# ecmwf/anemoi-models

Measured on AMD Instinct MI355X. Metric: mesh-node updates/sec (fwd step), higher is better.
Workload: dtype bf16; 1 GPU; N320->ico-6, 16 GT blocks, 1024 ch, batch 1, 2 x 90 input vars -> 80 output vars, full encoder+processor+decoder forward; mesh_nodes=40962, grid_nodes=542080, processor_blocks=16, rollout_steps=1, parallelism=single GPU, device=AMD Radeon Graphics

## Files before the change

anemoi_models_amd/_lib.py:

```python

from __future__ import annotations

import ctypes
import os
from ctypes import c_char_p
from ctypes import c_float
from ctypes import c_int
from ctypes import c_int64
from ctypes import c_uint32
from ctypes import c_void_p

import torch

_PKG_DIR = os.path.dirname(os.path.abspath(__file__))
LIB_PATH = os.path.join(_PKG_DIR, "lib", "libanemoi_amd.so")

ANEMOI_OK = 0
ANEMOI_ERR_INVALID = 1
ANEMOI_ERR_UNSUPPORTED = 2
ANEMOI_ERR_LAUNCH = 3

F32 = 0
BF16 = 1
I32 = 2
U8 = 3

ACT_NONE, ACT_GELU, ACT_SILU, ACT_RELU = 0, 1, 2, 3
ACT_CODES = {"Identity": ACT_NONE, "GELU": ACT_GELU, "SiLU": ACT_SILU, "ReLU": ACT_RELU}

LOSS_MSE, LOSS_MAE, LOSS_HUBER, LOSS_LOGCOSH = 0, 1, 2, 3
LOSS_KINDS = {"mse": LOSS_MSE, "mae": LOSS_MAE, "huber": LOSS_HUBER, "logcosh": LOSS_LOGCOSH}

ENS_AFCRPS, ENS_MEAN_SE, ENS_VARIANCE = 0, 1, 2
ENS_KINDS = {"afcrps": ENS_AFCRPS, "mean_se": ENS_MEAN_SE, "variance": ENS_VARIANCE}
ENS_MAX_MEMBERS = 16

COND_LN_MAX_K = 32


def cond_ln_padded_k(k: int) -> int:
    return 4 if k <= 4 else (8 if k <= 8 else (16 if k <= 16 else 32))


ABI_VERSION = 55

LINEAR_ENTRIES = {"linear": 0, "ln": 1, "stats": 2, "dual": 3, "actgrad": 4, "batched": 5}
LINEAR_KERNEL_NONE, LINEAR_KERNEL_128, LINEAR_KERNEL_PERSISTENT = 0, 1, 2
LINEAR_REST_NONE, LINEAR_REST_IN_LAUNCH, LINEAR_REST_SKINNY, LINEAR_REST_128 = 0, 1, 2, 3


class LinearArgs(ctypes.Structure):

    _fields_ = [
        ("struct_bytes", c_int64),
        ("entry", ctypes.c_int32), ("dtype", ctypes.c_int32), ("out_dtype", ctypes.c_int32), ("act", ctypes.c_int32),
        ("x", c_void_p), ("w", c_void_p), ("bias", c_void_p), ("colsum", c_void_p), ("stats", c_void_p),
        ("residual", c_void_p), ("y", c_void_p),
        ("ldx", c_int64), ("ldr", c_int64), ("ldy", c_int64), ("M", c_int64),
        ("N", ctypes.c_int32), ("K", ctypes.c_int32),
        ("workspace", c_void_p), ("workspace_bytes", c_int64), ("stats_out", c_void_p),
        ("stride_x", c_int64), ("stride_w", c_int64), ("stride_y", c_int64),
        ("batch", ctypes.c_int32), ("reserved", ctypes.c_int32),
    ]


class LinearRouteLaunch(ctypes.Structure):

    _fields_ = [
        ("row0", c_int64), ("rows", c_int64), ("tiles", c_int64),
        ("mh", ctypes.c_int32), ("blocks", ctypes.c_int32), ("tail_rows", ctypes.c_int32),
        ("stagger_phases", ctypes.c_int32), ("stagger_unit", ctypes.c_int32), ("reserved", ctypes.c_int32),
    ]


class LinearRoute(ctypes.Structure):

    _fields_ = [
        ("struct_bytes", c_int64),
        ("kernel", ctypes.c_int32), ("n_launches", ctypes.c_int32),
        ("launch", LinearRouteLaunch * 2),
        ("main_rows", c_int64),
        ("rest", ctypes.c_int32), ("nt", ctypes.c_int32),
        ("rest_row0", c_int64), ("rest_rows", c_int64), ("rs_rows", c_int64),
        ("vec_ok", ctypes.c_int32), ("split", ctypes.c_int32), ("model", ctypes.c_int32), ("reserved", ctypes.c_int32),
    ]


def linear_route(entry: str, **fields):
    args, route = LinearArgs(), LinearRoute()
    args.struct_bytes, route.struct_bytes = ctypes.sizeof(LinearArgs), ctypes.sizeof(LinearRoute)
    args.entry = LINEAR_ENTRIES[entry]
    for name, value in fields.items():
        setattr(args, name, value)
    return load().anemoi_linear_route(ctypes.byref(args), ctypes.byref(route)), route


class GtBlockArgs(ctypes.Structure):

    _fields_ = [
        ("struct_bytes", c_int64), ("n_dst", c_int64),
        ("dtype", ctypes.c_int32), ("C", ctypes.c_int32), ("H", ctypes.c_int32), ("up", ctypes.c_int32),
        ("hidden", ctypes.c_int32), ("act", ctypes.c_int32), ("k_proj", ctypes.c_int32), ("n_in", ctypes.c_int32),
        ("eps_mlp", c_float), ("eps_out", c_float),
        ("x", c_void_p), ("ldx", c_int64), ("x_stats", c_void_p),
        ("w_in", c_void_p), ("b_in", c_void_p), ("cs_in", c_void_p),
        ("sq", c_void_p), ("ld_sq", c_int64),
        ("q", c_void_p), ("k", c_void_p), ("v", c_void_p), ("x_r", c_void_p), ("u", c_void_p),
        ("ldq", c_int64), ("ldkv", c_int64), ("ldr", c_int64), ("ldu", c_int64),
        ("edge_attr", c_void_p), ("rowptr", c_void_p), ("col", c_void_p),
        ("att", c_void_p), ("ld_att", c_int64),
        ("w_proj", c_void_p), ("b_proj", c_void_p), ("res", c_void_p), ("ld_res", c_int64), ("y", c_void_p),
        ("y_stats", c_void_p),
        ("w_fc1", c_void_p), ("b_fc1", c_void_p), ("cs_fc1", c_void_p), ("h", c_void_p),
        ("w_fc2", c_void_p), ("b_fc2", c_void_p), ("out", c_void_p), ("out_stats", c_void_p),
        ("stats_ws", c_void_p), ("stats_ws_bytes", c_int64),
        ("run_ptr", c_void_p), ("run_perm", c_void_p), ("n_runs", c_int64),
        ("sched", c_void_p), ("sched_slots", ctypes.c_int32), ("sched_steps", ctypes.c_int32), ("n_src", c_int64),
        ("run_dst", c_void_p), ("n_edges", c_int64),
        ("tile_hdr", c_void_p), ("tile_dst", c_void_p), ("tile_src", c_void_p), ("tile_slot", c_void_p), ("tile_xcd", c_void_p),
        ("tile_max_per_xcd", ctypes.c_int32), ("tile_src_cap", ctypes.c_int32), ("tile_edge_cap", ctypes.c_int32),
        ("tile_pad", ctypes.c_int32),
    ]

class TfmBlockArgs(ctypes.Structure):

    _fields_ = [
        ("struct_bytes", c_int64), ("rows", c_int64),
        ("dtype", ctypes.c_int32), ("B", ctypes.c_int32), ("S", ctypes.c_int32), ("C", ctypes.c_int32), ("H", ctypes.c_int32),
        ("hidden", ctypes.c_int32), ("act", ctypes.c_int32), ("window", ctypes.c_int32),
        ("eps1", c_float), ("eps2", c_float),
        ("dropout_p", c_float), ("dropout_seed", c_uint32), ("dropout_seed_dev", c_void_p),
        ("dropout_h0", ctypes.c_int32), ("dropout_h_total", ctypes.c_int32),
        ("x", c_void_p), ("ldx", c_int64),
        ("ln1_w", c_void_p), ("ln1_b", c_void_p), ("ln2_w", c_void_p), ("ln2_b", c_void_p),
        ("w_qkv", c_void_p), ("b_qkv", c_void_p), ("w_proj", c_void_p), ("b_proj", c_void_p),
        ("w_fc1", c_void_p), ("b_fc1", c_void_p), ("w_fc2", c_void_p), ("b_fc2", c_void_p),
        ("h_ln", c_void_p), ("qkv", c_void_p), ("att", c_void_p), ("y", c_void_p), ("h", c_void_p),
        ("mhsa_ws", c_void_p), ("out", c_void_p),
    ]


OPT_MAX_TENSORS = 88
OPT_CHUNK = 4096
OPT_CONSTS = 8
OPT_SKIP_ALL = 3
OPT_SUMSQ_DEPTH = OPT_CHUNK // 256 + 6 + 3


class MultiTensorArgs(ctypes.Structure):

    _fields_ = [
        ("struct_bytes", c_int64), ("n_tensors", c_int64),
        ("numel", c_void_p), ("params", c_void_p), ("grads", c_void_p), ("exp_avg", c_void_p), ("exp_avg_sq", c_void_p),
        ("workspace", c_void_p), ("workspace_floats", c_int64), ("sumsq", c_void_p), ("consts", c_void_p), ("coef", c_void_p),
        ("beta1", ctypes.c_double), ("beta2", ctypes.c_double), ("eps", ctypes.c_double),
    ]


class AdamwConstantsArgs(ctypes.Structure):

    _fields_ = [
        ("struct_bytes", c_int64), ("n_groups", c_int64),
        ("step", c_void_p), ("lr_dev", c_void_p), ("lr", c_void_p), ("beta1", c_void_p), ("beta2", c_void_p),
        ("weight_decay", c_void_p), ("sumsq", c_void_p), ("skipped", c_void_p), ("consts", c_void_p),
        ("max_norm", c_float), ("has_max_norm", ctypes.c_int32), ("skip_nonfinite", ctypes.c_int32),
        ("reserved", ctypes.c_int32),
    ]


AVERAGE_EMA, AVERAGE_SWA = 0, 1
AVG_CONSTS = 4
LR_MAX_GROUPS = 32


class AverageConstantsArgs(ctypes.Structure):

    _fields_ = [
        ("struct_bytes", c_int64), ("n_averaged", c_void_p), ("step", c_void_p), ("skip", c_void_p), ("avg", c_void_p),
        ("decay", ctypes.c_double), ("start_step", c_int64), ("every", c_int64),
        ("kind", ctypes.c_int32), ("use_warmup", ctypes.c_int32),
    ]


class MultiAverageArgs(ctypes.Structure):

    _fields_ = [
        ("struct_bytes", c_int64), ("n_tensors", c_int64), ("numel", c_void_p), ("params", c_void_p), ("shadow", c_void_p),
        ("avg", c_void_p),
    ]


class MultiSwapArgs(ctypes.Structure):

    _fields_ = [("struct_bytes", c_int64), ("n_tensors", c_int64), ("numel", c_void_p), ("a", c_void_p), ("b", c_void_p)]


class LrScheduleArgs(ctypes.Structure):

    _fields_ = [
        ("struct_bytes", c_int64), ("n_groups", c_int64), ("step", c_void_p), ("lr", c_void_p), ("base", c_void_p),
        ("lr_min", c_void_p), ("warmup_start", c_void_p), ("warmup_steps", c_void_p), ("total_steps", c_void_p),
        ("warmup_prefix", c_void_p),
    ]


SIGNATURES = {
    "anemoi_abi_version": (c_int, []),
    "anemoi_build_info": (ctypes.c_char_p, []),
    "anemoi_last_error": (c_char_p, []),
    "anemoi_layer_norm": (c_int, [c_int, c_void_p, c_int64, c_void_p, c_void_p, c_void_p, c_int64, c_int64, c_int,
                                  c_float, c_void_p]),
    "anemoi_layer_norm_residual": (c_int, [c_int, c_void_p, c_int64, c_void_p, c_void_p, c_void_p, c_int64, c_void_p, c_int64,
                                           c_int64, c_int, c_float, c_void_p]),
    "anemoi_layer_norm_stats": (c_int, [c_int, c_void_p, c_int64, c_void_p, c_void_p, c_void_p, c_int64, c_void_p, c_int64,
                                        c_int, c_float, c_void_p]),
    "anemoi_linear": (c_int, [c_int, c_int, c_void_p, c_int64, c_void_p, c_void_p, c_void_p, c_int64, c_void_p,
                              c_int64, c_int64, c_int, c_int, c_int, c_void_p]),
    "anemoi_linear_stats": (c_int, [c_int, c_void_p, c_int64, c_void_p, c_void_p, c_void_p, c_void_p, c_void_p, c_int64,
                                    c_void_p, c_int64, c_int64, c_int, c_int, c_void_p, c_int64, c_float, c_void_p,
                                    c_void_p]),
    "anemoi_row_stats": (c_int, [c_int, c_void_p, c_int64, c_void_p, c_int64, c_int, c_float, c_void_p]),
    "anemoi_linear_ln": (c_int, [c_int, c_int, c_void_p, c_int64, c_void_p, c_void_p, c_void_p, c_void_p, c_void_p,
                                 c_int64, c_void_p, c_int64, c_int64, c_int, c_int, c_int, c_void_p]),
    "anemoi_edge_attr_csr": (c_int, [c_void_p, c_int, c_void_p, c_int, c_int64, c_void_p, c_void_p, c_int, c_int,
                                     c_int64, c_void_p]),
    "anemoi_gt_edge_attention_folded": (c_int, [c_int, c_void_p, c_int64, c_void_p, c_void_p, c_int64, c_void_p,
                                                c_int64, c_void_p, c_int64, c_void_p, c_int, c_void_p, c_void_p,
                                                c_void_p, c_int64, c_void_p, c_int64, c_int, c_int, c_void_p]),
    "anemoi_gt_edge_attention_raw": (c_int, [c_void_p, c_int64, c_void_p, c_int64, c_void_p, c_void_p, c_int64, c_void_p,
                                             c_int, c_void_p, c_void_p, c_void_p, c_int64, c_void_p, c_int64, c_int64,
                                             c_int, c_int, c_int, c_int, c_void_p]),
    "anemoi_gt_edge_attention_folded_runs": (c_int, [c_int, c_void_p, c_int64, c_void_p, c_void_p, c_int64, c_void_p,
                                                     c_int64, c_void_p, c_int64, c_void_p, c_int, c_void_p, c_void_p,
                                                     c_void_p, c_void_p, c_int64, c_void_p, c_int64, c_void_p, c_int64, c_int,
                                                     c_int, c_void_p]),
    "anemoi_gt_edge_attention_folded_groups": (c_int, [c_int, c_void_p, c_int64, c_void_p, c_void_p, c_int64, c_void_p,
                                                       c_int64, c_void_p, c_int64, c_void_p, c_int, c_void_p, c_void_p,
                                                       c_void_p, c_void_p, c_void_p, c_int64, c_int64, c_void_p, c_int64,
                                                       c_void_p, c_int64, c_int, c_int, c_void_p]),
    "anemoi_edge_schedule_shape": (c_int, [c_int, c_int64, c_int, c_void_p, c_void_p]),
    "anemoi_gt_edge_attention_folded_sched": (c_int, [c_int, c_void_p, c_int64, c_void_p, c_void_p, c_int64, c_void_p,
                                                      c_int64, c_void_p, c_int64, c_void_p, c_int, c_void_p, c_void_p,
                                                      c_void_p, c_int, c_int, c_int64, c_int64, c_void_p, c_int64, c_void_p,
                                                      c_int64, c_int, c_int, c_void_p]),
    "anemoi_gt_edge_attention_folded_tiles": (c_int, [c_int, c_void_p, c_int64, c_void_p, c_void_p, c_int64, c_void_p,
                                                      c_int64, c_void_p, c_int64, c_void_p, c_int, c_void_p, c_void_p,
                                                      c_void_p, c_void_p, c_void_p, c_void_p, c_void_p, c_int, c_int, c_int,
                                                      c_int64, c_int64, c_void_p, c_int64, c_void_p, c_int64, c_int, c_int,
                                                      c_void_p]),
    "anemoi_linear_dual": (c_int, [c_int, c_void_p, c_int64, c_void_p, c_void_p, c_void_p, c_int64, c_void_p, c_int64,
                                   c_int64, c_int, c_int, c_int, c_void_p]),
    "anemoi_linear_route": (c_int, [ctypes.POINTER(LinearArgs), ctypes.POINTER(LinearRoute)]),
    "anemoi_linear_actgrad": (c_int, [c_int, c_void_p, c_int64, c_void_p, c_void_p, c_int64, c_void_p, c_int64, c_int64,
                                      c_int, c_int, c_int, c_void_p]),
    "anemoi_gt_conv": (c_int, [c_int, c_void_p, c_int64, c_void_p, c_void_p, c_int64, c_void_p, c_int64, c_void_p, c_int64,
                               c_void_p, c_void_p, c_void_p, c_int64, c_void_p, c_int64, c_int, c_int, c_float, c_uint32,
                               c_void_p, c_void_p]),
    "anemoi_gt_conv_backward_dst": (c_int, [c_int, c_void_p, c_int64, c_void_p, c_void_p, c_int64, c_void_p, c_int64,
                                            c_void_p, c_int64, c_void_p, c_void_p, c_void_p, c_void_p, c_void_p, c_void_p,
                                            c_void_p, c_int64, c_int64, c_int, c_int, c_float, c_uint32, c_void_p,
                                            c_void_p]),
    "anemoi_gt_conv_backward_src": (c_int, [c_int, c_void_p, c_int64, c_void_p, c_int64, c_void_p, c_void_p, c_void_p,
                                            c_void_p, c_void_p, c_void_p, c_void_p, c_void_p, c_int64, c_void_p, c_int64,
                                            c_int64, c_int, c_int, c_float, c_uint32, c_void_p, c_void_p]),
    "anemoi_gt_edge_attention": (c_int, [c_int, c_void_p, c_int64, c_void_p, c_void_p, c_int64, c_void_p, c_int64,
                                         c_void_p, c_int, c_int, c_void_p, c_void_p, c_void_p, c_void_p, c_void_p,
                                         c_int64, c_int64, c_int, c_int, c_void_p]),
    "anemoi_gather_add_act": (c_int, [c_int, c_void_p, c_int64, c_void_p, c_int64, c_void_p, c_int64, c_void_p, c_void_p,
                                      c_void_p, c_int64, c_int64, c_int, c_int, c_void_p]),
    "anemoi_segment_sum": (c_int, [c_int, c_void_p, c_int64, c_void_p, c_void_p, c_int64, c_int64, c_int, c_void_p]),
    "anemoi_segment_sum_cat": (c_int, [c_int, c_void_p, c_int64, c_void_p, c_void_p, c_int64, c_void_p, c_int64, c_int64,
                                       c_int, c_void_p]),
    "anemoi_mhsa_workspace_bytes": (c_int64, [c_int, c_int, c_int, c_int, c_int]),
    "anemoi_mhsa": (c_int, [c_int, c_void_p, c_int64, c_void_p, c_int64, c_void_p, c_void_p, c_int, c_int, c_int, c_int,
                            c_int, c_float, c_uint32, c_void_p, c_int, c_int, c_void_p]),
    "anemoi_mhsa_backward_workspace_bytes": (c_int64, [c_int, c_int, c_int, c_int, c_int]),
    "anemoi_mhsa_backward": (c_int, [c_int, c_void_p, c_int64, c_void_p, c_int64, c_void_p, c_int64, c_void_p, c_void_p,
                                     c_void_p, c_int64, c_void_p, c_int, c_int, c_int, c_int, c_int, c_float, c_uint32,
                                     c_void_p, c_int, c_int, c_void_p]),
    "anemoi_assemble_nodes": (c_int, [c_int, c_void_p, c_int, c_int, c_int, c_int64, c_int, c_void_p, c_int,
                                      c_void_p, c_int, c_void_p, c_int64, c_void_p, c_void_p, c_void_p]),
    "anemoi_finalize_output": (c_int, [c_void_p, c_int, c_void_p, c_int, c_int, c_int, c_int64, c_int, c_void_p,
                                       c_void_p, c_void_p, c_void_p, c_void_p, c_void_p]),
    "anemoi_assemble_node_rows": (c_int, [c_int, c_void_p, c_int, c_int64, c_int, c_void_p, c_int, c_void_p, c_int,
                                          c_void_p, c_int64, c_void_p, c_int64, c_void_p, c_void_p, c_void_p]),
    "anemoi_finalize_output_rows": (c_int, [c_void_p, c_int, c_void_p, c_int, c_int64, c_int, c_void_p, c_void_p, c_int64,
                                            c_void_p, c_void_p, c_void_p, c_void_p, c_void_p]),
    "anemoi_bound_output": (c_int, [c_void_p, c_int, c_int64, c_int, c_void_p, c_void_p, c_void_p, c_void_p, c_int,
                                    c_void_p, c_void_p, c_void_p, c_void_p]),
    "anemoi_prognostic_residual": (c_int, [c_void_p, c_int, c_void_p, c_int, c_int, c_int, c_int64, c_int, c_void_p,
                                           c_void_p, c_int, c_void_p]),
    "anemoi_advance_input": (c_int, [c_void_p, c_int, c_int, c_int, c_int64, c_int, c_void_p, c_int, c_void_p, c_int,
                                     c_void_p, c_void_p]),
    "anemoi_advance_state": (c_int, [c_void_p, c_void_p, c_int, c_int, c_int, c_int64, c_int, c_void_p, c_int, c_void_p,
                                     c_int, c_void_p, c_void_p]),
    "anemoi_advance_state_backward": (c_int, [c_void_p, c_void_p, c_void_p, c_int, c_int, c_int, c_int64, c_int, c_int,
                                              c_void_p, c_void_p, c_int, c_void_p]),
    "anemoi_assemble_nodes_backward": (c_int, [c_int, c_void_p, c_int64, c_void_p, c_int, c_int, c_int, c_int64, c_int,
                                               c_void_p]),
    "anemoi_prognostic_residual_backward": (c_int, [c_void_p, c_int, c_void_p, c_int, c_int, c_int, c_int64, c_int,
                                                    c_void_p, c_void_p]),
    "anemoi_csr_project": (c_int, [c_void_p, c_int64, c_int64, c_int64, c_void_p, c_int64, c_int64, c_int64, c_int, c_int,
                                   c_int64, c_int64, c_void_p, c_void_p, c_void_p, c_void_p, c_void_p, c_int, c_void_p,
                                   c_void_p, c_int, c_void_p]),
    "anemoi_weighted_mse_workspace_floats": (c_int64, [c_int64, c_int]),
    "anemoi_weighted_mse": (c_int, [c_void_p, c_void_p, c_int64, c_int, c_int64, c_void_p, c_void_p, c_void_p, c_float,
                                    c_void_p, c_void_p, c_int64, c_void_p]),
    "anemoi_weighted_mse_backward": (c_int, [c_void_p, c_void_p, c_int64, c_int, c_int64, c_void_p, c_void_p, c_void_p,
                                             c_float, c_void_p, c_void_p, c_void_p]),
    "anemoi_weighted_error_workspace_floats": (c_int64, [c_int64, c_int64, c_int]),
    "anemoi_weighted_error": (c_int, [c_int, c_float, c_void_p, c_void_p, c_int64, c_int, c_int64, c_int64, c_void_p, c_void_p,
                                      c_void_p, c_void_p, c_float, c_void_p, c_void_p, c_int64, c_void_p]),
    "anemoi_weighted_error_backward": (c_int, [c_int, c_float, c_void_p, c_void_p, c_int64, c_int, c_int64, c_int64, c_void_p,
                                               c_void_p, c_void_p, c_void_p, c_float, c_void_p, c_void_p, c_void_p]),
    "anemoi_ensemble_score_workspace_floats": (c_int64, [c_int64, c_int64, c_int, c_int]),
    "anemoi_ensemble_score": (c_int, [c_int, c_float, c_void_p, c_void_p, c_int64, c_int, c_int64, c_int, c_int64, c_void_p,
                                      c_void_p, c_void_p, c_void_p, c_float, c_void_p, c_void_p, c_int64, c_void_p]),
    "anemoi_ensemble_score_backward": (c_int, [c_int, c_float, c_void_p, c_void_p, c_int64, c_int, c_int64, c_int, c_int64,
                                               c_void_p, c_void_p, c_void_p, c_void_p, c_float, c_void_p, c_void_p, c_void_p]),
    "anemoi_cond_layer_norm": (c_int, [c_int, c_void_p, c_int64, c_void_p, c_int64, c_int, c_void_p, c_int64, c_void_p, c_void_p,
                                       c_void_p, c_void_p, c_int64, c_void_p, c_int64, c_int, c_float, c_void_p]),
    "anemoi_cond_layer_norm_backward_workspace_floats": (c_int64, [c_int64, c_int, c_int]),
    "anemoi_cond_layer_norm_backward": (c_int, [c_int, c_void_p, c_int64, c_void_p, c_int64, c_void_p, c_void_p, c_int64, c_int,
                                                c_void_p, c_int64, c_void_p, c_void_p, c_void_p, c_int64, c_void_p, c_void_p, c_void_p,
                                                c_void_p, c_void_p, c_int64, c_int, c_void_p, c_int64, c_void_p]),
    "anemoi_gaussian_noise": (c_int, [c_void_p, c_int64, c_int, c_float, c_uint32, c_void_p, c_void_p]),
    "anemoi_transpose": (c_int, [c_int, c_void_p, c_int64, c_void_p, c_int64, c_int64, c_int, c_void_p]),
    "anemoi_transpose_colsum_rows": (c_int64, [c_int64, c_int64]),
    "anemoi_transpose_chunked": (c_int, [c_int, c_void_p, c_int64, c_void_p, c_int64, c_int64, c_int, c_int64, c_void_p,
                                         c_void_p]),
    "anemoi_weight_grad_tn": (c_int, [c_void_p, c_int64, c_void_p, c_int64, c_void_p, c_int64, c_void_p, c_int64, c_int64,
                                      c_int, c_int, c_int, c_void_p]),
    "anemoi_linear_batched": (c_int, [c_int, c_int, c_void_p, c_int64, c_int64, c_void_p, c_int64, c_void_p, c_int64,
                                      c_int64, c_int, c_int64, c_int, c_int, c_void_p]),
    "anemoi_col_sum_workspace_floats": (c_int64, [c_int64, c_int]),
# ... 97 lines not shown
```

anemoi_models_amd/layers/block.py:

```python

from __future__ import annotations

import os
from abc import ABC
from abc import abstractmethod
from typing import Optional

import torch
from torch import Tensor
from torch import nn

from .. import ops
from .. import runtime
from .. import training
from ..runtime import EdgePlan
from .conv import GraphConv
from .conv import GraphTransformerConv
from .mlp import MLP
from .mlp import NativeSequential
from .mlp import activation_class
from .mlp import fused_activation_name
from .mlp import linear_native
from .normalization import ConditionalLayerNorm


def inference_num_chunks() -> int:
    return int(os.environ.get("ANEMOI_INFERENCE_NUM_CHUNKS", "1"))


def _group_size(group) -> int:
    return 1 if group is None else group.size()


def _as_compute(x: Tensor, dtype: torch.dtype) -> Tensor:
    x = x if x.dtype == dtype else x.to(dtype)
    return x if (x.dim() == 2 and x.stride(1) == 1) else x.contiguous()



def folded_edge_phase(q: Tensor, k: Tensor, v: Tensor, x_r: Optional[Tensor], u: Tensor, edge_attr_csr: Tensor, plan,
                      num_heads: int, up: int, ld_out: Optional[int] = None) -> Tensor:
    lists = runtime.edge_lists(plan, q.dtype, q.shape[-1], num_heads, up)
    return ops.gt_edge_attention_folded(q, k, v, x_r, u, edge_attr_csr, plan.rowptr, plan.col, num_heads, up, ld_out=ld_out,
                                        **lists._asdict())


class EmbeddedRows:

    def __init__(self, x_aug: Tensor, one_col: int, emb: nn.Linear, h: Optional[Tensor], packed, tag: str) -> None:
        self.x_aug, self.one_col, self.emb, self.h, self._packed, self._tag = x_aug, one_col, emb, h, packed, tag

    @property
    def dtype(self) -> torch.dtype:
        return self.x_aug.dtype

    @property
    def device(self) -> torch.device:
        return self.x_aug.device

    @property
    def shape(self):
        return (self.x_aug.shape[0], self.emb.out_features)

    def stats(self, eps: float) -> Tensor:
        if self.h is not None:
            return ops.row_stats(self.h, eps)
        kp = self.x_aug.shape[1]
        t = self._packed.get((self._tag, "embstats", self.dtype, kp, self.one_col), [self.emb.weight, self.emb.bias],
                             lambda: runtime.embedding_stats_operator(self.emb.weight, self.emb.bias, kp, self.one_col,
                                                                      self.dtype))
        return ops.row_stats(runtime.linear(self.x_aug, t, None, stats_eps=eps), eps)


class BaseBlock(nn.Module, ABC):

    @abstractmethod
    def forward(self, x, edge_attr, edge_index, shapes, batch_size, size=None, model_comm_group=None): ...


class GraphTransformerBaseBlock(BaseBlock, ABC):

    def __init__(
        self,
        in_channels: int,
        hidden_dim: int,
        out_channels: int,
        edge_dim: int,
        num_heads: int = 16,
        bias: bool = True,
        activation: str = "GELU",
        num_chunks: int = 1,
        update_src_nodes: bool = False,
        **kwargs,
    ) -> None:
        super().__init__(**kwargs)
        self.update_src_nodes = update_src_nodes
        self.out_channels_conv = out_channels // num_heads
        self.num_heads = num_heads
        self.num_chunks = num_chunks
        self.activation = activation
        self.edge_dim = edge_dim
        width = num_heads * self.out_channels_conv

        self.lin_key = nn.Linear(in_channels, width)
        self.lin_query = nn.Linear(in_channels, width)
        self.lin_value = nn.Linear(in_channels, width)
        self.lin_self = nn.Linear(in_channels, width, bias=bias)
        self.lin_edge = nn.Linear(edge_dim, width)
        self.conv = GraphTransformerConv(out_channels=self.out_channels_conv)
        self.projection = nn.Linear(out_channels, out_channels)

        act = activation_class(activation)
        self.node_dst_mlp = nn.Sequential(
            nn.LayerNorm(out_channels), nn.Linear(out_channels, hidden_dim), act(), nn.Linear(hidden_dim, out_channels)
        )
        self.layer_norm1 = nn.LayerNorm(in_channels)
        if self.update_src_nodes:
            self.node_src_mlp = nn.Sequential(
                nn.LayerNorm(out_channels), nn.Linear(out_channels, hidden_dim), act(),
                nn.Linear(hidden_dim, out_channels),
            )
        self._packed = runtime.PackedWeights()
        self._plans = runtime.PlanCache()
        self._dst_mlp: Optional[NativeSequential] = None
        self._src_mlp: Optional[NativeSequential] = None

    def shard_qkve_heads(self, query: Tensor, key: Tensor, value: Tensor, edges: Tensor, shapes: tuple, batch_size: int,
                         model_comm_group=None):
        h, d = self.num_heads, self.out_channels_conv
        if _group_size(model_comm_group) <= 1:
            return tuple(t.reshape(t.shape[0], h, d) for t in (query, key, value, edges))
        from ..distributed.transformer import shard_heads

        assert batch_size == 1, "Only batch size of 1 is supported when model is sharded across GPUs"
        shapes_src, shapes_dst, shapes_edges = shapes
        out = []
        for t, shp in ((query, shapes_dst), (key, shapes_src), (value, shapes_src), (edges, shapes_edges)):
            t = t.reshape(1, t.shape[0], h, d).permute(0, 2, 1, 3)
            t = shard_heads(t, shapes=shp, mgroup=model_comm_group)
            out.append(t[0].permute(1, 0, 2).contiguous())
        return tuple(out)

    def shard_output_seq(self, out: Tensor, shapes: tuple, batch_size: int, model_comm_group=None) -> Tensor:
        if _group_size(model_comm_group) <= 1:
            return out.reshape(out.shape[0], -1)
        from ..distributed.transformer import shard_sequence

        t = out.permute(1, 0, 2).unsqueeze(0)
        t = shard_sequence(t, shapes=shapes[1], mgroup=model_comm_group)
        return t[0].permute(1, 0, 2).reshape(t.shape[2], -1).contiguous()

    def _cat_linear(self, tag: str, layers, dtype):
        w = self._packed.get((tag, "w", dtype), [l.weight for l in layers],
                             lambda: runtime.pack_weight([l.weight for l in layers], dtype))
# ... 405 lines not shown
            n_own = x_src.shape[0]
            kv = torch.empty((n_own + halo.n_recv, 2 * c), dtype=dtype, device=x_src.device)
            self._ln_linear(xs, *kv_args, out=kv[:n_own])
            pending = halo.start(kv, n_own)
        del xs
        xd = self._ln_begin(self.layer_norm2, x_dst)
        up = self.fold_width(dtype)
        if up is not None:
            wp, bp = self._folded_out(dtype, up)
            sq = self._ln_linear(xd, "squ", lambda: self._folded_in("squ", sq_layers, dtype, up),
                                 lambda: self._folded_rows(sq_layers, up),
                                 self._fold_params(sq_layers))
            del xd
            if halo is not None:
                halo.finish(pending)
            if num_chunks <= 1 and not self.update_src_nodes and not mx:
                new_dst = self._folded_tail(sq[:, c:2 * c], kv[:, :c], kv[:, c:], sq[:, :c], sq[:, 2 * c:], edge_attr_csr, plan,
                                            h_dst, up, out_stats_eps)
                return (x_src.h if isinstance(x_src, EmbeddedRows) else x_src), new_dst
            att = folded_edge_phase(sq[:, c:2 * c], kv[:, :c], kv[:, c:], sq[:, :c], sq[:, 2 * c:], edge_attr_csr, plan,
                                    self.num_heads, up, ld_out=wp.shape[1])
        else:
            if halo is not None:
                raise NotImplementedError("node-partitioned blocks need the folded edge kernel")
            wp, bp = self._cat_linear("proj", [self.projection], dtype)
            we, be = self._edge_params()
            sq = self._ln_linear(xd, "sq", lambda: self._cat_linear("sq", sq_layers, dtype),
                                 lambda: self._cat_rows(sq_layers),
                                 [l.weight for l in sq_layers] + [l.bias for l in sq_layers])
            del xd
            att = self.conv.fused(sq[:, c:], kv[:, :c], kv[:, c:], sq[:, :c], edge_attr_csr, self.edge_dim, we, be,
                                  plan, self.num_heads)
        del sq, kv
        y = runtime.linear(att, wp, bp, residual=h_dst,
                       stats_eps=self._mlp_ln_eps("dst", dtype) if num_chunks <= 1 else None)
        del att
        if mx:
            new_dst = self._mx_node_mlp(y, "dst", num_chunks)
        else:
            new_dst = self._node_mlp(y, "dst", num_chunks, out_stats_eps=out_stats_eps)
        if isinstance(x_src, EmbeddedRows):
            x_src = x_src.h
        new_src = self._node_mlp(x_src, "src", num_chunks) if self.update_src_nodes else x_src
        return new_src, new_dst

    RAW_ROWS_DEFAULT = "1"

    def _raw_source_weights(self, x_src, dtype):
        h, d = self.num_heads, self.out_channels_conv
        if (not isinstance(x_src, EmbeddedRows) or x_src.h is not None or self.update_src_nodes
                or dtype != torch.bfloat16 or not x_src.x_aug.is_cuda
                or os.environ.get("ANEMOI_AMD_EDGE_RAW", self.RAW_ROWS_DEFAULT) == "0"):
            return None
        ks, k_in = x_src.x_aug.shape[1], x_src.emb.in_features
        sum_col = ks - 1 if x_src.one_col != ks - 1 else ks - 2
        if self.fold_width(dtype) is None or h != 16 or ks not in (64, 128, 256) or sum_col < k_in:
            return None
        kv_layers = [self.lin_key, self.lin_value]
        ln, emb = self.layer_norm1, x_src.emb

        def build():
            f, b, _ = runtime.fold_embedded_layer_norm(*self._cat_rows(kv_layers), ln.weight, ln.bias, emb.weight,
                                                       emb.bias, ks, x_src.one_col, torch.float32)
            c = h * d
            w_qt = f[:c].view(h, d, ks).transpose(1, 2)
            w_g = f[c:].view(h, d, ks).clone()
            w_g[:, :, sum_col] = b[c:].view(h, d)
            if d % ops.k_multiple(dtype) != 0:
                w_qt, w_g = torch.block_diag(*w_qt), torch.block_diag(*w_g)
            return w_qt.to(dtype).contiguous(), w_g.to(dtype).contiguous(), sum_col

        return self._packed.get(("kv", "rawrows", dtype, ks, x_src.one_col, x_src._tag),
                                [l.weight for l in kv_layers] + [l.bias for l in kv_layers]
                                + [ln.weight, ln.bias, emb.weight, emb.bias], build)

    def _native_raw_sources(self, x_src, src_stats: Tensor, x_dst, h_dst: Tensor, edge_attr_csr: Tensor, plan, raw,
                            out_stats_eps: Optional[float]) -> Tensor:
        dtype = x_dst.dtype
        c, h = self.num_heads * self.out_channels_conv, self.num_heads
        w_qt, w_g, sum_col = raw
        up = self.fold_width(dtype)
        sq_layers = [self.lin_self, self.lin_query]
        wp, bp = self._folded_out(dtype, up)
        sq = self._ln_linear(self._ln_begin(self.layer_norm2, x_dst), "squ",
                             lambda: self._folded_in("squ", sq_layers, dtype, up),
                             lambda: self._folded_rows(sq_layers, up), self._fold_params(sq_layers))
        per_head = w_qt.dim() == 3
        qt = ops.linear_heads(sq[:, c:2 * c], w_qt) if per_head else runtime.linear(sq[:, c:2 * c], w_qt)
        att = torch.empty((sq.shape[0], wp.shape[1]), dtype=dtype, device=sq.device)
        if wp.shape[1] > c + h * up:
            att[:, c + h * up:].zero_()
        g = ops.gt_edge_attention_raw(qt, x_src.x_aug, src_stats, sq[:, 2 * c:2 * c + h * up], edge_attr_csr, plan.rowptr,
                                      plan.col, h, self.out_channels_conv, up, sum_col, att[:, c:c + h * up])
        del qt
        if per_head:
            ops.linear_heads(g, w_g, out=att[:, :c])
            ops.add(att[:, :c], sq[:, :c], out=att[:, :c])
        else:
            runtime.linear(g, w_g, residual=sq[:, :c], out=att[:, :c])
        del g
        del sq
        y = runtime.linear(att, wp, bp, residual=h_dst, stats_eps=self._mlp_ln_eps("dst", dtype))
        del att
        return self._node_mlp(y, "dst", 1, out_stats_eps=out_stats_eps)

    def _sharded(self, x, edge_attr: Tensor, edge_index: Tensor, shapes: tuple, batch_size: int, model_comm_group, size=None):
        from .. import autograd

        x_src, x_dst = x
        dtype = runtime.compute_dtype(x_dst)
        x_src, x_dst = _as_compute(x_src, dtype), _as_compute(x_dst, dtype)
        ln1, ln2 = self.layer_norm1, self.layer_norm2
        hs = autograd.layer_norm(x_src, ln1.weight, ln1.bias, ln1.eps)
        hd = autograd.layer_norm(x_dst, ln2.weight, ln2.bias, ln2.eps)
        x_r = autograd.linear(hd, self.lin_self.weight, self.lin_self.bias)
        q = autograd.linear(hd, self.lin_query.weight, self.lin_query.bias)
        k = autograd.linear(hs, self.lin_key.weight, self.lin_key.bias)
        v = autograd.linear(hs, self.lin_value.weight, self.lin_value.bias)
        e = autograd.linear(_as_compute(edge_attr, dtype), self.lin_edge.weight, self.lin_edge.bias)
        q, k, v, e = self.shard_qkve_heads(q, k, v, e, shapes, batch_size, model_comm_group)
        out = self.conv(q, k, v, e, edge_index, size=size)
        out = self.shard_output_seq(out, shapes, batch_size, model_comm_group)
        out = autograd.linear(out + x_r, self.projection.weight, self.projection.bias, "Identity", x_dst)
        new_src = training.sequential(self.node_src_mlp, x_src, residual=x_src) if self.update_src_nodes else x_src
        return new_src, training.sequential(self.node_dst_mlp, out, residual=out)

    def forward(
        self,
        x,
        edge_attr: Tensor,
        edge_index: Tensor,
        shapes: tuple,
        batch_size: int,
        model_comm_group=None,
        size=None,
    ):
        if _group_size(model_comm_group) > 1:
            assert batch_size == 1, "Only batch size of 1 is supported when model is sharded across GPUs"
            return self._sharded(x, edge_attr, edge_index, shapes, batch_size, model_comm_group, size), edge_attr
        if training.wants_grad(self, x[0], x[1], edge_attr):
            return training.gt_mapper_block(self, x, edge_attr, edge_index, size)
        x_src, x_dst = x
        dtype = runtime.compute_dtype(x_dst)
        n_src, n_dst = x_src.shape[0], x_dst.shape[0]
        if size is not None and tuple(size) != (n_src, n_dst):
            raise ValueError(f"Encountered tensors with sizes {(n_src, n_dst)}, but expected size {tuple(size)}")
        plan, ea = self._edge_inputs(edge_attr, edge_index, n_src, n_dst, dtype)
        num_chunks = self.num_chunks if self.training else inference_num_chunks()
        new_src, new_dst = self.native(_as_compute(x_src, dtype), _as_compute(x_dst, dtype), ea, plan, num_chunks)
        return (new_src if self.update_src_nodes else x[0], new_dst), edge_attr


class GraphConvBaseBlock(BaseBlock, ABC):
    def __init__(
        self,
        in_channels: int,
        out_channels: int,
        mlp_extra_layers: int = 0,
        activation: str = "SiLU",
        update_src_nodes: bool = True,
        num_chunks: int = 1,
        **kwargs,
    ) -> None:
        super().__init__(**kwargs)
        self.update_src_nodes = update_src_nodes
        self.num_chunks = num_chunks
        self.node_mlp = MLP(2 * in_channels, out_channels, out_channels, n_extra_layers=mlp_extra_layers,
                            activation=activation)
        self.conv = GraphConv(in_channels=in_channels, out_channels=out_channels, mlp_extra_layers=mlp_extra_layers,
                              activation=activation)
        self._packed = runtime.PackedWeights()
        self._plans = runtime.PlanCache()

    @abstractmethod
    def forward(self, x, edge_attr: Tensor, edge_index: Tensor, shapes: tuple, model_comm_group=None, size=None):
        """``(new nodes, new edge state)`` -- reference layers/block.py:157-167."""

    @staticmethod
    def _check_width(width: int, dtype) -> None:
        mult = ops.k_multiple(dtype)
# ... 307 lines not shown
```

anemoi_models_amd/layers/mapper.py:

```python

from __future__ import annotations

from abc import ABC
from typing import Optional

import numpy as np
import torch
from torch import Tensor
from torch import nn

from .. import ops
from .. import runtime
from .. import training
from .block import EmbeddedRows
from .block import GraphConvMapperBlock
from .block import GraphTransformerMapperBlock
from .block import inference_num_chunks
from .graph import TrainableTensor
from .mlp import MLP
from .mlp import linear_native


class BaseMapper(nn.Module, ABC):
    def __init__(self, in_channels_src: int = 0, in_channels_dst: int = 0, hidden_dim: int = 128,
# ... 31 lines not shown
        xin = x if x.dtype == dtype else x.to(dtype)
        return NativeSequential(seq)(xin if xin.stride(-1) == 1 else xin.contiguous())

    def pre_process(self, x, shard_shapes, model_comm_group=None):
        shapes_src, shapes_dst = shard_shapes
        x_src, x_dst = x
        return x_src, x_dst, shapes_src, shapes_dst

    def post_process(self, x_dst, shapes_dst, model_comm_group=None):
        return x_dst


class ForwardMapperPreProcessMixin:

    def pre_process(self, x, shard_shapes, model_comm_group=None):
        from ..distributed.shapes import change_channels_in_shape

        from ..distributed.graph import shard_tensor

        x_src, x_dst, shapes_src, shapes_dst = super().pre_process(x, shard_shapes, model_comm_group)
        x_src = shard_tensor(x_src, 0, shapes_src, model_comm_group)
        x_dst = shard_tensor(x_dst, 0, shapes_dst, model_comm_group)
        return (self._apply_module(self.emb_nodes_src, x_src), self._apply_module(self.emb_nodes_dst, x_dst),
                change_channels_in_shape(shapes_src, self.hidden_dim), change_channels_in_shape(shapes_dst, self.hidden_dim))


class BackwardMapperPostProcessMixin:

    def post_process(self, x_dst, shapes_dst, model_comm_group=None):
        from ..distributed.graph import gather_tensor
        from ..distributed.shapes import change_channels_in_shape

        x_dst = self._apply_module(self.node_data_extractor, x_dst)
        return gather_tensor(x_dst, 0, change_channels_in_shape(shapes_dst, self.out_channels_dst), model_comm_group)


class GraphEdgeMixin:

    def _register_edges(self, sub_graph, edge_attributes, src_size: int, dst_size: int, trainable_size: int) -> None:
        assert sub_graph, f"{self.__class__.__name__} needs a valid sub_graph to register edges."
        assert edge_attributes is not None, "Edge attributes must be provided"
        attr = torch.cat([sub_graph[name] for name in edge_attributes], dim=1)
        self.edge_dim = attr.shape[1] + trainable_size
        self.register_buffer("edge_attr", attr, persistent=False)
        self.register_buffer("edge_index_base", sub_graph.edge_index, persistent=False)
        self.register_buffer("edge_inc", torch.from_numpy(np.asarray([[src_size], [dst_size]], dtype=np.int64)),
                             persistent=True)

    def _expand_edges(self, edge_index: Tensor, edge_inc: Tensor, batch_size: int) -> Tensor:
        return runtime.expand_edges(edge_index, edge_inc, batch_size)


class GraphTransformerBaseMapper(GraphEdgeMixin, BaseMapper):
    def __init__(
        self,
        in_channels_src: int = 0,
        in_channels_dst: int = 0,
        hidden_dim: int = 128,
        trainable_size: int = 8,
        out_channels_dst: Optional[int] = None,
        num_chunks: int = 1,
        cpu_offload: bool = False,
        activation: str = "GELU",
        num_heads: int = 16,
        mlp_hidden_ratio: int = 4,
        sub_graph=None,
        sub_graph_edge_attributes: Optional[list] = None,
        src_grid_size: int = 0,
        dst_grid_size: int = 0,
    ) -> None:
        super().__init__(in_channels_src, in_channels_dst, hidden_dim, out_channels_dst=out_channels_dst,
                         num_chunks=num_chunks, cpu_offload=cpu_offload, activation=activation)
        self._register_edges(sub_graph, sub_graph_edge_attributes, src_grid_size, dst_grid_size, trainable_size)
        self.trainable = TrainableTensor(trainable_size=trainable_size, tensor_size=self.edge_attr.shape[0])
        self.proc = GraphTransformerMapperBlock(
            hidden_dim, mlp_hidden_ratio * hidden_dim, hidden_dim, num_heads=num_heads, edge_dim=self.edge_dim,
            activation=activation, num_chunks=num_chunks,
        )
        self.offload_layers(cpu_offload)
        self.emb_nodes_dst = nn.Linear(self.in_channels_dst, self.hidden_dim)
        self._packed = runtime.PackedWeights()
        self._plans = runtime.PlanCache()

    def _embed(self, x_src: Tensor, x_dst: Tensor, one_cols=(None, None)):
        return x_src, x_dst

    def _embedded(self, tag: str, lin: nn.Linear, x: Tensor, eps: Optional[float], one_col: Optional[int],
                  materialise: bool):
        k_in = lin.in_features
        if eps is None or not runtime.embed_fold_enabled(x.dtype) or 2 * (k_in + 1) > lin.out_features:
            return linear_native(self._packed, tag, lin, x, stats_eps=eps)
        if one_col is None:
            kp = ops.round_up(k_in + 1, ops.k_multiple(x.dtype))
            xa = torch.zeros((x.shape[0], kp), dtype=x.dtype, device=x.device)
            xa[:, :k_in].copy_(x[:, :k_in])
            xa[:, k_in].fill_(1.0)
            x, one_col = xa, k_in
        elif not (k_in <= one_col < x.shape[1]):
            raise ValueError(f"{tag}: constant-1 column {one_col} outside the K padding [{k_in}, {x.shape[1]})")
        h = linear_native(self._packed, tag, lin, x, stats_eps=eps) if materialise else None
        return EmbeddedRows(x, one_col, lin, h, self._packed, tag)

    def _extract(self, x_dst: Tensor, out_dtype) -> Tensor:
        return x_dst

    def _block_ln_eps(self, dtype):
        if not runtime.ln_fold_enabled(dtype):
            return None, None
        return self.proc.layer_norm1.eps, self.proc.layer_norm2.eps

    def _extract_ln_eps(self, dtype) -> Optional[float]:
        ext = getattr(self, "node_data_extractor", None)
        if isinstance(ext, nn.Sequential) and isinstance(ext[0], nn.LayerNorm) and runtime.ln_fold_enabled(dtype):
            return ext[0].eps
        return None

    def native(self, x_src: Tensor, x_dst: Tensor, batch_size: int, out_dtype: Optional[torch.dtype] = None,
               src_map: Optional[Tensor] = None, dst_map: Optional[Tensor] = None, one_cols=(None, None)) -> Tensor:
        n_src, n_dst = x_src.shape[0], x_dst.shape[0]
        plan = self._plans.get(self.edge_index_base, n_src, n_dst, batch_size, self.edge_inc, src_map, dst_map)
        ea = runtime.edge_attr_csr_cached(self._packed, self.edge_attr, self.trainable.trainable, plan,
                                          *self.proc.edge_layout(x_dst.dtype))
        h_src, h_dst = self._embed(x_src, x_dst, one_cols)
        num_chunks = self.proc.num_chunks if self.training else inference_num_chunks()
        _, h_dst = self.proc.native(h_src, h_dst, ea, plan, num_chunks, out_stats_eps=self._extract_ln_eps(h_dst.dtype))
        return self._extract(h_dst, out_dtype)

    def native_local(self, x_src: Tensor, x_dst: Tensor, local_graph, out_dtype: Optional[torch.dtype] = None,
                     one_cols=(None, None)) -> Tensor:
        plan = local_graph.plan
        ea = runtime.edge_attr_csr_cached(self._packed, self.edge_attr, self.trainable.trainable, plan,
                                          *self.proc.edge_layout(x_dst.dtype))
        h_src, h_dst = self._embed(x_src, x_dst, one_cols)
        num_chunks = self.proc.num_chunks if self.training else inference_num_chunks()
        _, h_dst = self.proc.native(h_src, h_dst, ea, plan, num_chunks, local_graph.halo,
                                    out_stats_eps=self._extract_ln_eps(h_dst.dtype))
        return self._extract(h_dst, out_dtype)

    def _run_sharded(self, x, batch_size: int, shard_shapes, model_comm_group) -> Tensor:
        from ..distributed.graph import shard_tensor
        from ..distributed.shapes import get_shape_shards

        size = (sum(s_[0] for s_ in shard_shapes[0]), sum(s_[0] for s_ in shard_shapes[1]))
        edge_attr = self.trainable(self.edge_attr, batch_size)
        edge_index = self._expand_edges(self.edge_index_base, self.edge_inc, batch_size)
        shapes_edge_attr = get_shape_shards(edge_attr, 0, model_comm_group)
        edge_attr = shard_tensor(edge_attr, 0, shapes_edge_attr, model_comm_group)
        x_src, x_dst, shapes_src, shapes_dst = self.pre_process(x, shard_shapes, model_comm_group)
        (x_src, x_dst), edge_attr = self.proc((x_src, x_dst), edge_attr, edge_index, (shapes_src, shapes_dst, shapes_edge_attr),
                                              batch_size, model_comm_group, size=size)
        return self.post_process(x_dst, shapes_dst, model_comm_group)

    def _run(self, x, batch_size: int, shard_shapes, model_comm_group) -> Tensor:
        if model_comm_group is not None and model_comm_group.size() > 1:
            assert batch_size == 1, "Only batch size of 1 is supported when model is sharded across GPUs"
            return self._run_sharded(x, batch_size, shard_shapes, model_comm_group)
        x_src, x_dst = x
        if shard_shapes is not None:
            size = (sum(s[0] for s in shard_shapes[0]), sum(s[0] for s in shard_shapes[1]))
            if size != (x_src.shape[0], x_dst.shape[0]):
                raise ValueError(f"shard_shapes describe {size} nodes, inputs have {(x_src.shape[0], x_dst.shape[0])}")
        if training.wants_grad(self, x_src, x_dst):
            with self._offloaded():
                return training.gt_mapper(self, x_src, x_dst, batch_size)
        dtype = runtime.compute_dtype(x_dst)

        def prep(t):
            t = t if t.dtype == dtype else t.to(dtype)
            return t if t.stride(-1) == 1 else t.contiguous()

        return self.native(prep(x_src), prep(x_dst), batch_size)

    def forward(self, x, batch_size: int, shard_shapes, model_comm_group=None) -> Tensor:
        return self._run(x, batch_size, shard_shapes, model_comm_group)


class GraphTransformerForwardMapper(ForwardMapperPreProcessMixin, GraphTransformerBaseMapper):

    def __init__(self, in_channels_src: int = 0, in_channels_dst: int = 0, hidden_dim: int = 128,
                 trainable_size: int = 8, out_channels_dst: Optional[int] = None, num_chunks: int = 1,
                 cpu_offload: bool = False, activation: str = "GELU", num_heads: int = 16, mlp_hidden_ratio: int = 4,
                 sub_graph=None, sub_graph_edge_attributes: Optional[list] = None, src_grid_size: int = 0,
                 dst_grid_size: int = 0) -> None:
        super().__init__(in_channels_src, in_channels_dst, hidden_dim, trainable_size,
                         out_channels_dst=out_channels_dst, num_chunks=num_chunks, cpu_offload=cpu_offload,
                         activation=activation, num_heads=num_heads, mlp_hidden_ratio=mlp_hidden_ratio,
                         sub_graph=sub_graph, sub_graph_edge_attributes=sub_graph_edge_attributes,
                         src_grid_size=src_grid_size, dst_grid_size=dst_grid_size)
        self.emb_nodes_src = nn.Linear(self.in_channels_src, self.hidden_dim)

    def _embed(self, x_src: Tensor, x_dst: Tensor, one_cols=(None, None)):
        eps1, eps2 = self._block_ln_eps(x_src.dtype)
        return (self._embedded("emb_nodes_src", self.emb_nodes_src, x_src, eps1, one_cols[0],
                               materialise=self.proc.update_src_nodes),
                self._embedded("emb_nodes_dst", self.emb_nodes_dst, x_dst, eps2, one_cols[1], materialise=True))

    def forward(self, x, batch_size: int, shard_shapes, model_comm_group=None):
        x_dst = self._run(x, batch_size, shard_shapes, model_comm_group)
        return x[0], x_dst


class GraphTransformerBackwardMapper(BackwardMapperPostProcessMixin, GraphTransformerBaseMapper):

    def __init__(self, in_channels_src: int = 0, in_channels_dst: int = 0, hidden_dim: int = 128,
                 trainable_size: int = 8, out_channels_dst: Optional[int] = None, num_chunks: int = 1,
                 cpu_offload: bool = False, activation: str = "GELU", num_heads: int = 16, mlp_hidden_ratio: int = 4,
                 sub_graph=None, sub_graph_edge_attributes: Optional[list] = None, src_grid_size: int = 0,
                 dst_grid_size: int = 0) -> None:
        super().__init__(in_channels_src, in_channels_dst, hidden_dim, trainable_size,
                         out_channels_dst=out_channels_dst, num_chunks=num_chunks, cpu_offload=cpu_offload,
                         activation=activation, num_heads=num_heads, mlp_hidden_ratio=mlp_hidden_ratio,
                         sub_graph=sub_graph, sub_graph_edge_attributes=sub_graph_edge_attributes,
                         src_grid_size=src_grid_size, dst_grid_size=dst_grid_size)
        self.node_data_extractor = nn.Sequential(nn.LayerNorm(self.hidden_dim),
                                                 nn.Linear(self.hidden_dim, self.out_channels_dst))
        self.proc.mx_node_mlp = False

    def pre_process(self, x, shard_shapes, model_comm_group=None):
        from ..distributed.shapes import change_channels_in_shape

        from ..distributed.graph import shard_tensor

        x_src, x_dst, shapes_src, shapes_dst = super().pre_process(x, shard_shapes, model_comm_group)
        x_dst = shard_tensor(x_dst, 0, shapes_dst, model_comm_group)
        return (x_src, self._apply_module(self.emb_nodes_dst, x_dst), change_channels_in_shape(shapes_src, self.hidden_dim),
                change_channels_in_shape(shapes_dst, self.hidden_dim))

    def _embed(self, x_src: Tensor, x_dst: Tensor, one_cols=(None, None)):
        return x_src, self._embedded("emb_nodes_dst", self.emb_nodes_dst, x_dst, self._block_ln_eps(x_dst.dtype)[1],
                                     one_cols[1], materialise=True)

    def _extract(self, x_dst: Tensor, out_dtype) -> Tensor:
        ln, lin = self.node_data_extractor[0], self.node_data_extractor[1]
        if runtime.ln_fold_enabled(x_dst.dtype) and x_dst.shape[1] % ops.k_multiple(x_dst.dtype) == 0:
            wf, bf, cs = self._packed.get(("extract", "lnfold", x_dst.dtype), [lin.weight, lin.bias, ln.weight, ln.bias],
                                          lambda: runtime.fold_layer_norm(lin.weight.detach().float(), lin.bias,
                                                                          ln.weight, ln.bias, x_dst.dtype))
            return runtime.linear(x_dst, wf, bf, out_dtype=out_dtype, ln=(ops.row_stats(x_dst, ln.eps), cs))
        h = ops.layer_norm(x_dst, runtime.f32c(ln.weight), runtime.f32c(ln.bias), ln.eps)
        return linear_native(self._packed, "extract", lin, h, out_dtype=out_dtype)

    def forward(self, x, batch_size: int, shard_shapes, model_comm_group=None) -> Tensor:
        return self._run(x, batch_size, shard_shapes, model_comm_group)


class GNNBaseMapper(GraphEdgeMixin, BaseMapper):
    def __init__(self, in_channels_src: int = 0, in_channels_dst: int = 0, hidden_dim: int = 128,
                 trainable_size: int = 8, out_channels_dst: Optional[int] = None, num_chunks: int = 1,
                 cpu_offload: bool = False, activation: str = "SiLU", mlp_extra_layers: int = 0, sub_graph=None,
                 sub_graph_edge_attributes: Optional[list] = None, src_grid_size: int = 0,
                 dst_grid_size: int = 0) -> None:
        super().__init__(in_channels_src, in_channels_dst, hidden_dim, out_channels_dst=out_channels_dst,
                         num_chunks=num_chunks, cpu_offload=cpu_offload, activation=activation)
        self._register_edges(sub_graph, sub_graph_edge_attributes, src_grid_size, dst_grid_size, trainable_size)
        self.emb_edges = MLP(in_features=self.edge_dim, hidden_dim=hidden_dim, out_features=hidden_dim,
                             n_extra_layers=mlp_extra_layers, activation=activation)
        self.trainable = TrainableTensor(trainable_size=trainable_size, tensor_size=self.edge_attr.shape[0])
        self._plans = runtime.PlanCache()

    def prepare_edges(self, size, batch_size: int, model_comm_group=None):
        from ..distributed.graph import shard_tensor
        from ..distributed.khop_edges import sort_edges_1hop_sharding

        edge_attr = self.trainable(self.edge_attr, batch_size)
        edge_index = self._expand_edges(self.edge_index_base, self.edge_inc, batch_size)
        if model_comm_group is not None and model_comm_group.size() > 1:
            edge_attr, edge_index, shapes_edge_attr, shapes_edge_idx = sort_edges_1hop_sharding(size, edge_attr, edge_index,
                                                                                                model_comm_group)
            edge_index = shard_tensor(edge_index, 1, shapes_edge_idx, model_comm_group)
            edge_attr = shard_tensor(edge_attr, 0, shapes_edge_attr, model_comm_group)
        return self.emb_edges(edge_attr), edge_index

    def _embed(self, x_src: Tensor, x_dst: Tensor):
        return x_src, x_dst

    def _extract(self, x_dst: Tensor, out_dtype) -> Tensor:
        return x_dst

    def native(self, x_src: Tensor, x_dst: Tensor, batch_size: int, out_dtype: Optional[torch.dtype] = None,
               src_map: Optional[Tensor] = None, dst_map: Optional[Tensor] = None):
        n_src, n_dst = x_src.shape[0], x_dst.shape[0]
        plan = self._plans.get(self.edge_index_base, n_src, n_dst, batch_size, self.edge_inc, src_map, dst_map)
        dtype = x_dst.dtype
        ea = ops.edge_attr_csr(self.edge_attr, self.trainable.trainable, plan.perm)
        e = ops.convert_pad(ea[:, : self.edge_dim], dtype, ops.round_up(self.edge_dim, ops.k_multiple(dtype)))
        e = self.emb_edges.native()(e)
        h_src, h_dst = self._embed(x_src, x_dst)
        (h_src, h_dst), _ = self.proc.native(h_src, h_dst, e, plan)
        return h_src, self._extract(h_dst, out_dtype)

    def native_local(self, x_src: Tensor, x_dst: Tensor, local_graph, out_dtype: Optional[torch.dtype] = None,
                     x_src_extra: Optional[Tensor] = None):
        plan = local_graph.plan
        dtype = x_dst.dtype
        ea = ops.edge_attr_csr(self.edge_attr, self.trainable.trainable, plan.perm)
        e = ops.convert_pad(ea[:, : self.edge_dim], dtype, ops.round_up(self.edge_dim, ops.k_multiple(dtype)))
        e = self.emb_edges.native()(e)
        h_src, h_dst = self._embed(x_src, x_dst)
        (_, h_dst), _ = self.proc.native(h_src, h_dst, e, plan, local_graph.halo)
        extra = None
        if x_src_extra is not None:
            hx = self.emb_nodes_src.native()(x_src_extra) if hasattr(self, "emb_nodes_src") else x_src_extra
            c = hx.shape[1]
            if self.proc.update_src_nodes:
                xcat = torch.empty((hx.shape[0], 2 * c), dtype=dtype, device=hx.device)
                xcat[:, :c].copy_(hx)
                xcat[:, c:].copy_(hx)
                hx = self.proc.node_mlp.native()(xcat, residual=hx)
            extra = hx
        return extra, self._extract(h_dst, out_dtype)

    def _run(self, x, batch_size: int, shard_shapes, model_comm_group):
        if model_comm_group is not None and model_comm_group.size() > 1:
            assert batch_size == 1, "Only batch size of 1 is supported when model is sharded across GPUs"
            size = (sum(s_[0] for s_ in shard_shapes[0]), sum(s_[0] for s_ in shard_shapes[1]))
            edge_attr, edge_index = self.prepare_edges(size, batch_size, model_comm_group)
            x_src, x_dst, shapes_src, shapes_dst = self.pre_process(x, shard_shapes, model_comm_group)
            (x_src, x_dst), _ = self.proc((x_src, x_dst), edge_attr, edge_index, (shapes_src, shapes_dst), model_comm_group,
                                          size=size)
            return x_src, self.post_process(x_dst, shapes_dst, model_comm_group)
        x_src, x_dst = x
# ... 68 lines not shown
```

anemoi_models_amd/models/encoder_processor_decoder.py:

```python

from __future__ import annotations

import logging
from typing import Optional

import torch
from torch import Tensor
from torch import nn

from .. import ops
from .. import runtime
from ..layers.graph import NamedNodesAttributes
from ..layers.truncation import project_add

try:
    from hydra.utils import instantiate as _hydra_instantiate
except ImportError:
    _hydra_instantiate = None

from ..utils.config import instantiate as _local_instantiate
from ..utils.config import REFERENCE_PREFIX

LOGGER = logging.getLogger(__name__)


def instantiate(cfg, **kwargs):
    target = cfg.get("_target_", "") if hasattr(cfg, "get") else ""
    if _hydra_instantiate is not None and not target.startswith(REFERENCE_PREFIX):
        return _hydra_instantiate(cfg, **kwargs)
    return _local_instantiate(cfg, **kwargs)


class AnemoiModelEncProcDec(nn.Module):

    def __init__(self, *, model_config, data_indices, graph_data, truncation_data=None) -> None:
        super().__init__()
        self._graph_data = graph_data
        self._graph_name_data = model_config.graph.data
        self._graph_name_hidden = model_config.graph.hidden

        self._calculate_shapes_and_indices(data_indices)
        self._assert_matching_indices(data_indices)
        self.data_indices = data_indices

        self.multi_step = model_config.training.multistep_input
        self.num_channels = model_config.model.num_channels

        self.node_attributes = NamedNodesAttributes(model_config.model.trainable_parameters.hidden, self._graph_data)
        data, hidden = self._graph_name_data, self._graph_name_hidden
        input_dim = self.multi_step * self.num_input_channels + self.node_attributes.attr_ndims[data]

        self.encoder = instantiate(
            model_config.model.encoder,
            in_channels_src=input_dim,
            in_channels_dst=self.node_attributes.attr_ndims[hidden],
            hidden_dim=self.num_channels,
            sub_graph=self._graph_data[(data, "to", hidden)],
            src_grid_size=self.node_attributes.num_nodes[data],
            dst_grid_size=self.node_attributes.num_nodes[hidden],
        )
        self.processor = instantiate(
            model_config.model.processor,
            num_channels=self.num_channels,
            sub_graph=self._graph_data[(hidden, "to", hidden)],
            src_grid_size=self.node_attributes.num_nodes[hidden],
            dst_grid_size=self.node_attributes.num_nodes[hidden],
            **self._processor_kwargs(model_config),
        )
        self.decoder = instantiate(
            model_config.model.decoder,
            in_channels_src=self.num_channels,
            in_channels_dst=input_dim,
            hidden_dim=self.num_channels,
            out_channels_dst=self.num_output_channels,
            sub_graph=self._graph_data[(hidden, "to", data)],
            src_grid_size=self.node_attributes.num_nodes[hidden],
            dst_grid_size=self.node_attributes.num_nodes[data],
        )
        self.boundings = nn.ModuleList(
            [
                instantiate(cfg, name_to_index=self.data_indices.internal_model.output.name_to_index)
                for cfg in getattr(model_config.model, "bounding", [])
            ]
        )
        self._idx_cache: dict = {}
        self._set_truncation(truncation_data)

    def _set_truncation(self, truncation_data) -> None:
        from ..layers.truncation import TruncationPlan

        plan = TruncationPlan(truncation_data, grid_size=self.node_attributes.num_nodes[self._graph_name_data])
        if plan and len(set(torch.as_tensor(self._internal_input_idx).tolist())) != len(self._internal_input_idx):
            raise ValueError("truncation_data: the prognostic input columns repeat (the input gradient stores each column once)")
        self._truncation = plan if plan else None

    def _calculate_shapes_and_indices(self, data_indices) -> None:
        self.num_input_channels = len(data_indices.internal_model.input)
        self.num_output_channels = len(data_indices.internal_model.output)
        self._internal_input_idx = data_indices.internal_model.input.prognostic
        self._internal_output_idx = data_indices.internal_model.output.prognostic

    def _assert_matching_indices(self, data_indices) -> None:
        n_full = len(data_indices.internal_model.output.full)
        n_diag = len(data_indices.internal_model.output.diagnostic)
        assert len(self._internal_output_idx) == n_full - n_diag, (
            f"Mismatch between the internal data indices ({len(self._internal_output_idx)}) and "
            f"the internal output indices excluding diagnostic variables ({n_full - n_diag})"
        )
        assert len(self._internal_input_idx) == len(
            self._internal_output_idx
        ), f"Internal model indices must match {self._internal_input_idx} != {self._internal_output_idx}"

    def _run_mapper(self, mapper: nn.Module, data, batch_size: int, shard_shapes, model_comm_group=None,
                    use_reentrant: bool = False):
        kwargs = dict(batch_size=batch_size, shard_shapes=shard_shapes, model_comm_group=model_comm_group)
        if not torch.is_grad_enabled():
            return mapper(data, **kwargs)
        from torch.utils.checkpoint import checkpoint

        return checkpoint(mapper, data, **kwargs, use_reentrant=use_reentrant)

    def _processor_kwargs(self, model_config) -> dict:
        return {}

    def _processor_condition(self, batch_size: int, x_latent: Tensor) -> Optional[Tensor]:
        return None

    def _prognostic_indices(self, device):
        key = str(device)
        if key not in self._idx_cache:
            as_i32 = lambda t: torch.as_tensor(t).to(device=device, dtype=torch.int32).contiguous()
            self._idx_cache[key] = (as_i32(self._internal_output_idx), as_i32(self._internal_input_idx))
        return self._idx_cache[key]

    def _mesh_order(self, device):
        key = ("mesh_order", str(device))
        if key not in self._idx_cache:
            latlons = self.node_attributes.latlons(self._graph_name_hidden)
            if not getattr(self, "mesh_locality_order", True):
                order = torch.arange(latlons.shape[0], device=device)
            else:
                order = runtime.locality_order(latlons).to(device)
            self._idx_cache[key] = (order, runtime.inverse_permutation(order))
        return self._idx_cache[key]

    def _with_ones(self, trainable: Optional[Tensor], n_nodes: int, enabled: bool, device=None) -> Optional[Tensor]:
        if not enabled:
            return trainable
        device = trainable.device if trainable is not None else (device or self.node_attributes.latlons(
            self._graph_name_data).device)
        key = ("ones", n_nodes, str(device))
        if key not in self._idx_cache:
            self._idx_cache[key] = torch.ones((n_nodes, 1), dtype=torch.float32, device=device)
        ones = self._idx_cache[key]
        return ones if trainable is None else torch.cat([trainable.detach().float(), ones], dim=1)

    def _embed_fold(self, dtype: torch.dtype) -> bool:
        from ..layers.mapper import GraphTransformerBaseMapper

        return (runtime.embed_fold_enabled(dtype) and isinstance(self.encoder, GraphTransformerBaseMapper)
                and isinstance(self.decoder, GraphTransformerBaseMapper))

    @staticmethod
    def _feature_ld(width: int, dtype: torch.dtype, wide: bool = True) -> int:
        ld = ops.round_up(width, ops.k_multiple(dtype))
        return max(ld, 128) if (wide and dtype == torch.bfloat16) else ld

    @staticmethod
# ... 21 lines not shown
        elif key not in self._idx_cache:
            src = torch.full((self.num_output_channels,), -1, dtype=torch.int32)
            src[torch.as_tensor(self._internal_output_idx).long()] = torch.as_tensor(self._internal_input_idx).to(torch.int32)
            self._idx_cache[key] = src.to(y.device)
        if len(self.boundings) == 0:
            ops.finalize_output(y, x, self._idx_cache[key], input_affine, output_affine, rows=rows)
            return y if y.dtype == out_dtype else y.to(out_dtype)
        plan = self._bounding_plan(y.device, output_affine)
        if plan is None:
            ops.finalize_output(y, x, self._idx_cache[key], input_affine, None, rows=rows)
            if y.dtype != out_dtype:
                y = y.to(out_dtype)
            for bounding in self.boundings:
                y = bounding(y)
            if output_affine is not None:
                y = (y - output_affine[1]) / output_affine[0]
            return y
        op_lists, masked_affine, fin = plan
        ops.finalize_output(y, x, self._idx_cache[key], input_affine, masked_affine, rows=rows)
        ops.bound_output(y, *op_lists, fin=fin)
        return y if y.dtype == out_dtype else y.to(out_dtype)

    def _bounding_plan(self, device, output_affine):
        from ..layers.bounding import bounded_columns
        from ..layers.bounding import compile_boundings

        key = ("boundings", str(device), None if output_affine is None else
               (output_affine[0].data_ptr(), output_affine[0]._version, output_affine[1].data_ptr(),
                output_affine[1]._version))
        if key not in self._idx_cache:
            op_list = compile_boundings(self.boundings)
            if op_list is None:
                self._idx_cache[key] = None
                return None
            lists = (torch.tensor([o[0] for o in op_list], dtype=torch.int32, device=device),
                     torch.tensor([o[1] for o in op_list], dtype=torch.float32, device=device),
                     torch.tensor([o[2] for o in op_list], dtype=torch.float32, device=device),
                     torch.tensor([o[3] for o in op_list], dtype=torch.int32, device=device))
            masked = fin = None
            if output_affine is not None:
                cols = torch.tensor(bounded_columns(op_list), dtype=torch.int64, device=device)
                mul, add = (t.detach().to(device=device, dtype=torch.float32).contiguous() for t in output_affine)
                m_mul, m_add = mul.clone(), add.clone()
                m_mul[cols] = 1.0
                m_add[cols] = 0.0
                masked = (m_mul, m_add)
                fin = (cols.to(torch.int32), mul[cols].contiguous(), add[cols].contiguous())
            self._idx_cache[key] = (lists, masked, fin)
        return self._idx_cache[key]

    def _training_forward(self, x: Tensor, input_affine=None, output_affine=None) -> Tensor:
        from .. import training

        if input_affine is not None or output_affine is not None:
            raise NotImplementedError("input_affine / output_affine belong to the inference interface (predict_step)")
        return training.model_forward(self, x)

    def forward(self, x: Tensor, model_comm_group=None, *, input_affine=None, output_affine=None) -> Tensor:
        if model_comm_group is not None and model_comm_group.size() > 1:
            from ..distributed.partition import sharded_forward

            if getattr(self, "_truncation", None) is not None:
                from ..layers.truncation import REFUSAL

                raise NotImplementedError(REFUSAL)
            return sharded_forward(self, x, model_comm_group, input_affine=input_affine, output_affine=output_affine)
        if torch.is_grad_enabled() and any(p.requires_grad for p in self.parameters()):
            return self._training_forward(x, input_affine, output_affine)
        runtime.require_inference(self)
        batch_size, _, ensemble_size, grid, _ = x.shape
        dtype = runtime.compute_dtype(x)
        kmult = ops.k_multiple(dtype)
        data, hidden = self._graph_name_data, self._graph_name_hidden
        na = self.node_attributes

        width = self.multi_step * self.num_input_channels + na.attr_ndims[data]
        fold = self._embed_fold(dtype)
        tr_data = na.trainable_tensors[data].trainable
        x_data = ops.assemble_nodes(x, na.latlons(data), self._with_ones(tr_data, grid, fold), batch_size, dtype,
                                    ld_out=self._feature_ld(width + int(fold), dtype, fold), in_affine=input_affine)
        order, inv = self._mesh_order(x.device)
        tr_hidden = na.trainable_tensors[hidden].trainable
        w_hidden = na.attr_ndims[hidden]
        x_hidden = ops.assemble_nodes(None, na.latlons(hidden)[order],
                                      self._with_ones(None if tr_hidden is None else tr_hidden[order], order.numel(), fold),
                                      batch_size, dtype, ld_out=self._feature_ld(w_hidden + int(fold), dtype, fold))
        one_data, one_hidden = (width, w_hidden) if fold else (None, None)

        enc = self.encoder.native(x_data, x_hidden, batch_size, dst_map=inv,
                                  **self._one_cols(self.encoder, one_data, one_hidden))
        x_data_latent, x_latent = (x_data, enc) if not isinstance(enc, tuple) else enc
        cond = self._processor_condition(batch_size, x_latent)
        x_proc = (self.processor.native(x_latent, batch_size, node_map=inv) if cond is None
                  else self.processor.native(x_latent, batch_size, node_map=inv, cond=cond))
        x_latent_proc = ops.add(x_proc, x_latent)
        y = self.decoder.native(x_latent_proc, x_data_latent, batch_size, out_dtype=torch.float32, src_map=inv,
                                **self._one_cols(self.decoder, None, one_data if x_data_latent is x_data else None))
        if isinstance(y, tuple):
            y = y[1]

        y = y.view(batch_size, ensemble_size, grid, self.num_output_channels)
        return self._finish(y, x, input_affine, output_affine)
```

anemoi_models_amd/ops.py:

```python

from __future__ import annotations

from typing import NamedTuple
from typing import Optional

import torch
from torch import Tensor

from . import _lib

_DT = {torch.float32: _lib.F32, torch.bfloat16: _lib.BF16}

PROFILE: Optional[list] = None


class _Timed:
    __slots__ = ("name", "work", "start")

    def __init__(self, name: str, **work) -> None:
        self.name, self.work, self.start = name, work, None

    def __enter__(self):
        if PROFILE is not None:
            self.start = torch.cuda.Event(enable_timing=True)
            self.start.record(torch.cuda.current_stream())
        return self

    def __exit__(self, *exc):
        if self.start is not None:
            end = torch.cuda.Event(enable_timing=True)
            end.record(torch.cuda.current_stream())
            PROFILE.append((self.name, self.start, end, self.work))
        return False


def dtype_code(dtype: torch.dtype) -> int:
    try:
        return _DT[dtype]
    except KeyError:
        raise NotImplementedError(f"compute dtype {dtype} is not supported (float32 or bfloat16)") from None


def k_multiple(dtype: torch.dtype) -> int:
    return 128 // torch.empty((), dtype=dtype).element_size()


def round_up(n: int, m: int) -> int:
    return (n + m - 1) // m * m


def _dev(*tensors: Optional[Tensor]) -> None:
    for t in tensors:
        if t is not None and not t.is_cuda:
            raise RuntimeError(
                "anemoi_models_amd kernels run on an MI355X only: got a CPU tensor (there is no CPU fallback)"
            )


_raw_stream = getattr(torch._C, "_cuda_getCurrentRawStream", None)


def _stream() -> int:
    if _raw_stream is not None:
        return _raw_stream(torch.cuda.current_device())
    return torch.cuda.current_stream().cuda_stream


def _rows(t: Tensor) -> Tensor:
    if t.dim() != 2 or (t.shape[1] > 1 and t.stride(1) != 1):
        raise ValueError(f"expected a row-major 2-D tensor (unit inner stride), got shape {tuple(t.shape)} "
                         f"strides {t.stride()}")
    return t


def _ld(t: Tensor) -> int:
    return t.stride(0) if t.shape[0] > 1 else max(t.stride(0), t.shape[1])


def _ptr(t: Optional[Tensor]) -> Optional[int]:
    return None if t is None else t.data_ptr()


def layer_norm(x: Tensor, weight: Tensor, bias: Tensor, eps: float = 1e-5, out: Optional[Tensor] = None,
               residual: Optional[Tensor] = None) -> Tensor:
    _dev(x, weight, bias, out, residual)
    _rows(x)
    if out is None:
        out = torch.empty((x.shape[0], x.shape[1]), dtype=x.dtype, device=x.device)
    if residual is not None and (residual.dtype != x.dtype or residual.shape != x.shape):
        raise ValueError("layer_norm: the residual must have the shape and dtype of x")
    if x.shape[0] == 0:
        return out
    if residual is not None:
        with _Timed("layer_norm", bytes=3 * x.shape[0] * x.shape[1] * x.element_size()):
            st = _lib.load().anemoi_layer_norm_residual(dtype_code(x.dtype), x.data_ptr(), _ld(x), weight.data_ptr(),
                                                        bias.data_ptr(), residual.data_ptr(), _ld(_rows(residual)),
                                                        out.data_ptr(), _ld(_rows(out)), x.shape[0], x.shape[1], eps, _stream())
        _lib.check(st, "anemoi_layer_norm_residual")
        return out
    with _Timed("layer_norm", bytes=2 * x.shape[0] * x.shape[1] * x.element_size()):
        st = _lib.load().anemoi_layer_norm(dtype_code(x.dtype), x.data_ptr(), _ld(x), weight.data_ptr(),
                                           bias.data_ptr(), out.data_ptr(), _ld(_rows(out)), x.shape[0], x.shape[1],
                                           eps, _stream())
    _lib.check(st, "anemoi_layer_norm")
    return out


def layer_norm_with_stats(x: Tensor, weight: Tensor, bias: Tensor, eps: float = 1e-5):
    _dev(x, weight, bias)
    _rows(x)
    out = torch.empty((x.shape[0], x.shape[1]), dtype=x.dtype, device=x.device)
    stats = torch.empty((x.shape[0], 2), dtype=torch.float32, device=x.device)
# ... 264 lines not shown
    if rowptr.dtype != torch.int32 or col.dtype != torch.int32 or rowptr.shape[0] != n_dst + 1:
        raise ValueError("gt_edge_attention: rowptr/col must be int32 with rowptr of length n_dst + 1")
    if col.shape[0] == 0:
        col = torch.zeros(1, dtype=torch.int32, device=q.device)
        edge_attr = torch.zeros((1, max(4, round_up(edge_dim, 4))), dtype=torch.float32, device=q.device)
    alg_bytes = (2 * n_dst + 2 * k.shape[0]) * c * q.element_size() + col.shape[0] * 52 + (n_dst + 1) * 4
    with _Timed("gt_edge_attention", bytes=alg_bytes, n_dst=n_dst, n_src=k.shape[0], edges=col.shape[0]):
        st = _lib.load().anemoi_gt_edge_attention(
            dtype_code(q.dtype), q.data_ptr(), _ld(q), k.data_ptr(), v.data_ptr(), _ld(k), _ptr(x_r),
            0 if x_r is None else _ld(_rows(x_r)), edge_attr.data_ptr(),
            edge_attr.stride(0) if edge_attr.shape[0] > 1 else edge_attr.shape[1], edge_dim, w_edge.data_ptr(),
            b_edge.data_ptr(), rowptr.data_ptr(), col.data_ptr(), out.data_ptr(), _ld(_rows(out)), n_dst, c,
            num_heads, _stream())
    _lib.check(st, "anemoi_gt_edge_attention")
    return out


def gt_edge_attention_folded(q: Tensor, k: Tensor, v: Tensor, x_r: Optional[Tensor], u: Tensor, edge_attr: Tensor,
                             rowptr: Tensor, col: Tensor, num_heads: int, up: int, out: Optional[Tensor] = None,
                             ld_out: Optional[int] = None, lse: Optional[Tensor] = None, runs=None, sched=None,
                             tiles=None) -> Tensor:
    _dev(q, k, v, x_r, u, edge_attr, rowptr, col, out, lse)
    if lse is not None and (lse.dtype != torch.float32 or not lse.is_contiguous()
                            or tuple(lse.shape) != (_rows(q).shape[0], num_heads)):
        raise ValueError("gt_edge_attention_folded: lse must be a contiguous f32 [n_dst, H] tensor")
    n_dst, c = _rows(q).shape
    if _ld(_rows(k)) != _ld(_rows(v)):
        raise ValueError("gt_edge_attention_folded: k and v must share their leading dimension")
    width = c + num_heads * up
    ld = width if ld_out is None else ld_out
    if out is None:
        out = torch.empty((n_dst, ld), dtype=q.dtype, device=q.device)
        if ld > width:
            out[:, width:].zero_()
    if rowptr.dtype != torch.int32 or col.dtype != torch.int32 or rowptr.shape[0] != n_dst + 1:
        raise ValueError("gt_edge_attention_folded: rowptr/col must be int32 with rowptr of length n_dst + 1")
    if edge_attr.shape[0] != col.shape[0] or (col.shape[0] > 0 and (edge_attr.shape[1] != up or
                                                                      not edge_attr.is_contiguous())):
        raise ValueError("gt_edge_attention_folded: edge_attr must be contiguous [E, up]")
    if col.shape[0] == 0:
        col = torch.zeros(1, dtype=torch.int32, device=q.device)
        edge_attr = torch.zeros((1, up), dtype=torch.float32, device=q.device)
    alg_bytes = (2 * n_dst + 2 * k.shape[0]) * c * q.element_size() + col.shape[0] * 52 + (n_dst + 1) * 4
    fused_bytes = alg_bytes + n_dst * ((0 if x_r is None else c) + 2 * num_heads * up) * q.element_size()
    with _Timed("gt_edge_attention", bytes=alg_bytes, fused_bytes=fused_bytes, n_dst=n_dst, n_src=k.shape[0], edges=col.shape[0]):
        lib = _lib.load()
        head = (dtype_code(q.dtype), q.data_ptr(), _ld(q), k.data_ptr(), v.data_ptr(), _ld(_rows(k)), _ptr(x_r),
                0 if x_r is None else _ld(_rows(x_r)), u.data_ptr(), _ld(_rows(u)), edge_attr.data_ptr(), up,
                rowptr.data_ptr(), col.data_ptr())
        tail = (out.data_ptr(), _ld(_rows(out)), _ptr(lse), n_dst, c, num_heads, _stream())
        n_src, n_edges = _rows(k).shape[0], col.shape[0]
        if runs is not None and len(runs) == 3:
            grp_ptr, grp_perm, grp_dst = runs
            _dev(grp_ptr, grp_perm, grp_dst)
            if (grp_ptr.dtype != torch.int32 or grp_perm.dtype != torch.int32 or grp_dst.dtype != torch.int32
                    or grp_perm.shape[0] != n_dst or grp_dst.shape[0] != n_dst):
                raise ValueError("gt_edge_attention_folded: runs = (int32 grp_ptr [n_groups + 1], int32 grp_perm [n_dst], "
                                 "int32 grp_dst [n_dst])")
            st = lib.anemoi_gt_edge_attention_folded_groups(*head, grp_ptr.data_ptr(), grp_dst.data_ptr(), grp_perm.data_ptr(),
                                                            grp_ptr.shape[0] - 1, n_src, *tail)
        elif runs is not None:
            run_ptr, perm = runs
            _dev(run_ptr, perm)
            if run_ptr.dtype != torch.int32 or perm.dtype != torch.int32 or perm.shape[0] != run_ptr.shape[0] - 1:
                raise ValueError("gt_edge_attention_folded: runs = (int32 run_ptr [n_runs + 1], int32 perm [n_runs])")
            st = lib.anemoi_gt_edge_attention_folded_runs(*head, run_ptr.data_ptr(), perm.data_ptr(), run_ptr.shape[0] - 1, *tail)
        elif tiles is not None:
            _dev(tiles.hdr, tiles.dst, tiles.src, tiles.slot, tiles.xcd)
            st = lib.anemoi_gt_edge_attention_folded_tiles(
                *head, tiles.hdr.data_ptr(), tiles.dst.data_ptr(), tiles.src.data_ptr(), tiles.slot.data_ptr(),
                tiles.xcd.data_ptr(), tiles.max_tiles_per_xcd, tiles.src_cap, tiles.edge_cap, n_src, n_edges, *tail)
        elif sched is not None:
            _dev(sched)
            if sched.dtype != torch.int32 or sched.dim() != 3 or sched.shape[0] != 8 or not sched.is_contiguous():
                raise ValueError("gt_edge_attention_folded: sched = contiguous int32 [8, slots, steps]")
            st = lib.anemoi_gt_edge_attention_folded_sched(*head, sched.data_ptr(), sched.shape[1], sched.shape[2], n_src,
                                                           n_edges, *tail)
        else:
            st = lib.anemoi_gt_edge_attention_folded(*head, *tail)
    _lib.check(st, "anemoi_gt_edge_attention_folded")
    return out


def linear_heads(x: Tensor, w: Tensor, out: Optional[Tensor] = None) -> Tensor:
    _dev(x, w, out)
    _rows(x)
    if w.dim() != 3 or w.dtype != x.dtype or not w.is_contiguous():
        raise ValueError("linear_heads: weight must be contiguous [H, N, K] in the activation dtype")
    h, n, k = w.shape
    if x.shape[1] < h * k:
        raise ValueError(f"linear_heads: x has {x.shape[1]} columns, {h} heads of {k} expected")
    if out is None:
        out = torch.empty((x.shape[0], h * n), dtype=x.dtype, device=x.device)
    if _rows(out).shape[1] < h * n or out.dtype != x.dtype or out.shape[0] != x.shape[0]:
        raise ValueError("linear_heads: out must be [M, >= H*N] in the activation dtype")
    m = x.shape[0]
    if m == 0:
        return out
    code = dtype_code(x.dtype)
    with _Timed("linear", flops=2 * m * h * n * k, bytes=(m * h * (k + n) + h * n * k) * x.element_size(), m=m, n=h * n,
                k=k, heads=h):
        st = _lib.load().anemoi_linear_batched(code, code, x.data_ptr(), _ld(x), k, w.data_ptr(), n * k, out.data_ptr(),
                                               _ld(out), n, h, m, n, k, _stream())
    _lib.check(st, "anemoi_linear_batched")
    return out


def gt_edge_attention_raw(qt: Tensor, x_raw: Tensor, src_stats: Tensor, u: Tensor, edge_attr: Tensor, rowptr: Tensor,
                          col: Tensor, num_heads: int, head_dim: int, up: int, sum_col: int, t_out: Tensor,
                          g: Optional[Tensor] = None) -> Tensor:
    _dev(qt, x_raw, src_stats, u, edge_attr, rowptr, col, t_out, g)
    n_dst, ks = _rows(qt).shape[0], _rows(x_raw).shape[1]
    if qt.dtype != torch.bfloat16 or x_raw.dtype != torch.bfloat16 or u.dtype != torch.bfloat16 or t_out.dtype != torch.bfloat16:
        raise NotImplementedError("gt_edge_attention_raw: bf16 only")
    if qt.shape[1] != num_heads * ks:
        raise ValueError(f"gt_edge_attention_raw: qt has {qt.shape[1]} columns, {num_heads} heads of {ks} expected")
    if (src_stats.shape != (x_raw.shape[0], 2) or src_stats.dtype != torch.float32 or not src_stats.is_contiguous()):
        raise ValueError("gt_edge_attention_raw: src_stats must be the contiguous [n_src, 2] f32 result of row_stats")
    if rowptr.dtype != torch.int32 or col.dtype != torch.int32 or rowptr.shape[0] != n_dst + 1:
        raise ValueError("gt_edge_attention_raw: rowptr/col must be int32 with rowptr of length n_dst + 1")
    if edge_attr.shape[0] != col.shape[0] or (col.shape[0] > 0 and (edge_attr.shape[1] != up or
                                                                      not edge_attr.is_contiguous())):
        raise ValueError("gt_edge_attention_raw: edge_attr must be contiguous [E, up]")
    if _rows(u).shape != (n_dst, num_heads * up) or _rows(t_out).shape[0] != n_dst or t_out.shape[1] < num_heads * up:
        raise ValueError("gt_edge_attention_raw: u / t_out must be [n_dst, H*up]")
    if g is None:
        g = torch.empty((n_dst, num_heads * ks), dtype=qt.dtype, device=qt.device)
    if col.shape[0] == 0:
        col = torch.zeros(1, dtype=torch.int32, device=qt.device)
        edge_attr = torch.zeros((1, up), dtype=torch.float32, device=qt.device)
    alg_bytes = (col.shape[0] * (ks * 2 + 4 + up * 4 + 4) + 2 * n_dst * num_heads * ks * 2 + (n_dst + 1) * 4)
    fused_bytes = alg_bytes + n_dst * 2 * num_heads * up * 2
    with _Timed("gt_edge_attention", bytes=alg_bytes, fused_bytes=fused_bytes, n_dst=n_dst, n_src=x_raw.shape[0],
                edges=col.shape[0], raw_rows=ks):
        st = _lib.load().anemoi_gt_edge_attention_raw(
            qt.data_ptr(), _ld(qt), x_raw.data_ptr(), _ld(x_raw), src_stats.data_ptr(), u.data_ptr(), _ld(u),
            edge_attr.data_ptr(), up, rowptr.data_ptr(), col.data_ptr(), g.data_ptr(), _ld(_rows(g)), t_out.data_ptr(),
            _ld(t_out), n_dst, num_heads, ks, head_dim, sum_col, _stream())
    _lib.check(st, "anemoi_gt_edge_attention_raw")
    return g


def gt_conv(q: Tensor, k: Tensor, v: Tensor, edges_csr: Tensor, rowptr: Tensor, col: Tensor, num_heads: int,
            x_r: Optional[Tensor] = None, lse: Optional[Tensor] = None, dropout_p: float = 0.0, dropout_seed: int = 0,
            seed_dev: Optional[Tensor] = None) -> Tensor:
    if not 0.0 <= dropout_p <= 1.0:
        raise ValueError(f"dropout probability has to be between 0 and 1, but got {dropout_p}")
    _dev(q, k, v, edges_csr, rowptr, col, x_r, lse)
    n_dst, c = _rows(q).shape
    if _ld(_rows(k)) != _ld(_rows(v)):
        raise ValueError("gt_conv: k and v must share their leading dimension")
    if rowptr.dtype != torch.int32 or col.dtype != torch.int32 or rowptr.shape[0] != n_dst + 1:
        raise ValueError("gt_conv: rowptr/col must be int32 with rowptr of length n_dst + 1")
    if edges_csr.shape[0] != col.shape[0] or edges_csr.dtype != q.dtype:
        raise ValueError("gt_conv: edges must be [E, C] in the activation dtype")
    out = torch.empty((n_dst, c), dtype=q.dtype, device=q.device)
    if col.shape[0] == 0:
        if lse is not None:
            lse.fill_(float("-inf"))
        return out.zero_() if x_r is None else out.copy_(x_r)
    alg_bytes = (2 * n_dst + 2 * k.shape[0] + col.shape[0]) * c * q.element_size() + col.shape[0] * 4 + (n_dst + 1) * 4
    with _Timed("gt_conv", bytes=alg_bytes, n_dst=n_dst, n_src=k.shape[0], edges=col.shape[0]):
        st = _lib.load().anemoi_gt_conv(dtype_code(q.dtype), q.data_ptr(), _ld(q), k.data_ptr(), v.data_ptr(), _ld(_rows(k)),
                                        edges_csr.data_ptr(), _ld(_rows(edges_csr)), _ptr(x_r),
                                        0 if x_r is None else _ld(_rows(x_r)), rowptr.data_ptr(), col.data_ptr(),
                                        out.data_ptr(), _ld(out), _ptr(lse), n_dst, c, num_heads, float(dropout_p),
                                        int(dropout_seed) & 0xFFFFFFFF, _seed_dev_ptr(seed_dev, q), _stream())
    _lib.check(st, "anemoi_gt_conv")
    return out


def gather_add_act(t: Tensor, p_dst: Tensor, p_src: Tensor, dst: Tensor, src: Tensor, act: str = "Identity",
                   out: Optional[Tensor] = None) -> Tensor:
    _dev(t, p_dst, p_src, dst, src, out)
    e, c = _rows(t).shape
    if out is None:
        out = torch.empty((e, c), dtype=t.dtype, device=t.device)
    if e == 0:
        return out
    if dst.dtype != torch.int32 or src.dtype != torch.int32 or dst.shape[0] != e or src.shape[0] != e:
        raise ValueError("gather_add_act: dst / src must be int32 [E]")
    with _Timed("gather_add_act", bytes=(2 * e + p_dst.shape[0] + p_src.shape[0]) * c * t.element_size() + 8 * e):
        st = _lib.load().anemoi_gather_add_act(dtype_code(t.dtype), t.data_ptr(), _ld(t), p_dst.data_ptr(),
                                               _ld(_rows(p_dst)), p_src.data_ptr(), _ld(_rows(p_src)), dst.data_ptr(),
                                               src.data_ptr(), out.data_ptr(), _ld(_rows(out)), e, c,
                                               _lib.ACT_CODES[act], _stream())
    _lib.check(st, "anemoi_gather_add_act")
    return out
# ... 486 lines not shown
    return dpred


def _ens_args(who: str, pred: Tensor, target: Tensor, row_w: Tensor, kind: str, n_members: int, alpha: float,
              col_w: Optional[Tensor], mask: Optional[Tensor], diff_scale: Optional[Tensor], n_groups: int,
              upstream: Optional[Tensor] = None):
    rows, v, g, n_groups = _loss_operands(who, pred, target, row_w, col_w, mask, diff_scale, n_groups, ensemble=True,
                                          upstream=upstream)
    if kind not in _lib.ENS_KINDS:
        raise ValueError(f"{who}: unknown kind {kind!r} (one of {sorted(_lib.ENS_KINDS)})")
    e = int(n_members)
    if e < 2:
        raise ValueError(f"{who}: an ensemble score needs at least 2 members, got n_members = {e}")
    if e > _lib.ENS_MAX_MEMBERS:
        raise NotImplementedError(f"{who}: n_members = {e}, at most {_lib.ENS_MAX_MEMBERS}")
    if not 0.0 <= float(alpha) <= 1.0:
        raise ValueError(f"{who}: alpha must lie in [0, 1], got {alpha}")
    if pred.shape[1] != v or pred.shape[0] != rows * e:
        raise ValueError(f"{who}: pred {tuple(pred.shape)} is not [rows * n_members, V] of target {tuple(target.shape)} with "
                         f"n_members = {e}")
    return rows, v, g, e, n_groups, _lib.ENS_KINDS[kind]


def ensemble_score(pred: Tensor, target: Tensor, row_w: Tensor, kind: str, *, n_members: int, alpha: float = 1.0,
                   col_w: Optional[Tensor] = None, mask: Optional[Tensor] = None, diff_scale: Optional[Tensor] = None,
                   n_groups: int = 1, scale: float = 1.0) -> Tensor:
    rows, v, g, e, n_groups, code = _ens_args("ensemble_score", pred, target, row_w, kind, n_members, alpha, col_w, mask,
                                              diff_scale, n_groups)
    out = torch.empty((n_groups, v), dtype=torch.float32, device=target.device)
    return _loss_forward("ensemble_score", (n_groups, rows // n_groups, v, e), (code, float(alpha)), pred, target,
                         (rows, v, g, e, n_groups, row_w.data_ptr(), _ptr(col_w), _ptr(mask), _ptr(diff_scale), float(scale)), out)


def ensemble_score_backward(pred: Tensor, target: Tensor, row_w: Tensor, kind: str, *, n_members: int, alpha: float = 1.0,
                            col_w: Optional[Tensor] = None, mask: Optional[Tensor] = None,
                            diff_scale: Optional[Tensor] = None, n_groups: int = 1, scale: float = 1.0,
                            upstream: Tensor) -> Tensor:
    rows, v, g, e, n_groups, code = _ens_args("ensemble_score_backward", pred, target, row_w, kind, n_members, alpha, col_w,
                                              mask, diff_scale, n_groups, upstream)
    dpred = torch.empty_like(pred)
    if rows == 0 and code == _lib.ENS_AFCRPS:
        return dpred
    with _Timed("ensemble_score_backward", bytes=(2 * pred.numel() + target.numel()) * 4):
        st = _lib.load().anemoi_ensemble_score_backward(code, float(alpha), _ptr(pred) or upstream.data_ptr(),
                                                        _ptr(target) or upstream.data_ptr(), rows, v, g, e, n_groups,
                                                        row_w.data_ptr(), _ptr(col_w), _ptr(mask), _ptr(diff_scale),
                                                        float(scale), upstream.data_ptr(), dpred.data_ptr(), _stream())
    _lib.check(st, "anemoi_ensemble_score_backward")
    return dpred


def prognostic_residual(y: Tensor, x: Tensor, out_idx: Tensor, in_idx: Tensor) -> Tensor:
    _dev(y, x, out_idx, in_idx)
    if y.dtype != torch.float32 or not y.is_contiguous():
        raise ValueError("prognostic_residual: y must be contiguous float32")
    b, t, ens, g, v_in = x.shape
    x = x.contiguous().float()
    st = _lib.load().anemoi_prognostic_residual(y.data_ptr(), y.shape[-1], x.data_ptr(), b, t, ens, g, v_in,
                                                out_idx.data_ptr(), in_idx.data_ptr(), out_idx.shape[0], _stream())
    _lib.check(st, "anemoi_prognostic_residual")
    return y


def convert_pad(src: Tensor, dtype: torch.dtype, ld_out: Optional[int] = None) -> Tensor:
    _dev(src)
    _rows(src)
    rows, cols = src.shape
    ld = cols if ld_out is None else ld_out
    out = torch.empty((rows, ld), dtype=dtype, device=src.device)
    if rows == 0:
        return out
    st = _lib.load().anemoi_convert_pad(dtype_code(src.dtype), src.data_ptr(), _ld(src), dtype_code(dtype),
                                        out.data_ptr(), ld, rows, cols, _stream())
    _lib.check(st, "anemoi_convert_pad")
    return out


def add(a: Tensor, b: Tensor, out: Optional[Tensor] = None) -> Tensor:
    _dev(a, b, out)
    if a.shape != b.shape or a.dtype != b.dtype:
        raise ValueError("add: shape / dtype mismatch")
    if out is None:
        out = torch.empty(a.shape, dtype=a.dtype, device=a.device)
    st = _lib.load().anemoi_add(dtype_code(a.dtype), a.data_ptr(), _ld(_rows(a)), b.data_ptr(), _ld(_rows(b)),
                                out.data_ptr(), _ld(_rows(out)), a.shape[0], a.shape[1], _stream())
    _lib.check(st, "anemoi_add")
    return out


def transpose(x: Tensor, ld_out: Optional[int] = None) -> Tensor:
    _dev(x)
    rows, cols = _rows(x).shape
    ld = rows if ld_out is None else ld_out
    out = torch.empty((cols, ld), dtype=x.dtype, device=x.device)
    st = _lib.load().anemoi_transpose(dtype_code(x.dtype), x.data_ptr(), _ld(x), out.data_ptr(), ld, rows, cols, _stream())
    _lib.check(st, "anemoi_transpose")
    return out


def col_sum(x: Tensor, out: Optional[Tensor] = None) -> Tensor:
    _dev(x)
    rows, cols = _rows(x).shape
    lib = _lib.load()
    if out is None:
        out = torch.empty(cols, dtype=torch.float32, device=x.device)
    elif out.dtype != torch.float32 or out.numel() != cols or not out.is_contiguous():
        raise ValueError("col_sum: out must be a contiguous f32 vector of the column count")
    if rows == 0:
        return out.zero_()
    n_ws = lib.anemoi_col_sum_workspace_floats(rows, cols)
    ws = torch.empty(max(n_ws, 1), dtype=torch.float32, device=x.device)
    st = lib.anemoi_col_sum(dtype_code(x.dtype), x.data_ptr(), _ld(x), rows, cols, out.data_ptr(), ws.data_ptr(), n_ws,
                            _stream())
    _lib.check(st, "anemoi_col_sum")
    return out


def row_dot(a: Tensor, b: Tensor, shift: Optional[Tensor] = None) -> Tensor:
    _dev(a, b, shift)
    rows, cols = _rows(a).shape
    if tuple(_rows(b).shape) != (rows, cols) or a.dtype != b.dtype:
        raise ValueError("row_dot: a and b must have the same shape and dtype")
    if shift is not None and (shift.dtype != torch.float32 or shift.numel() < cols or not shift.is_contiguous()):
        raise ValueError("row_dot: shift must be a contiguous f32 vector with one entry per column")
    out = torch.empty(rows, dtype=torch.float32, device=a.device)
    with _Timed("row_dot", bytes=2 * rows * cols * a.element_size()):
        st = _lib.load().anemoi_row_dot(dtype_code(a.dtype), a.data_ptr(), _ld(_rows(a)), b.data_ptr(), _ld(_rows(b)),
                                        _ptr(shift), out.data_ptr(), rows, cols, _stream())
    _lib.check(st, "anemoi_row_dot")
    return out


def row_scale(x: Tensor, s: Tensor, alpha: float = 1.0, out: Optional[Tensor] = None) -> Tensor:
    _dev(x, s, out)
    rows, cols = _rows(x).shape
    if s.dtype != torch.float32 or s.numel() != rows or not s.is_contiguous():
        raise ValueError("row_scale: s must be a contiguous f32 vector with one entry per row")
    if out is None:
        out = torch.empty((rows, cols), dtype=x.dtype, device=x.device)
    with _Timed("row_scale", bytes=2 * rows * cols * x.element_size()):
        st = _lib.load().anemoi_row_scale(dtype_code(x.dtype), x.data_ptr(), _ld(_rows(x)), s.data_ptr(), float(alpha),
                                          out.data_ptr(), _ld(_rows(out)), rows, cols, _stream())
    _lib.check(st, "anemoi_row_scale")
    return out


def _fused_epilogue_rows(dtype, m: int, n: int, k: int, ldx: int, ldp: int = 0) -> int:
    if not (dtype == torch.bfloat16 and n >= 256 and n % 8 == 0 and k >= 128 and k % 64 == 0 and ldx % 8 == 0 and ldp % 8 == 0):
        return 0
    m_main = (m // 256) * 256
    if m_main < 1024:
        return 0
    return m if m - m_main <= 8 else m_main


def linear_dual(x: Tensor, w: Tensor, bias: Optional[Tensor], act: str):
    _dev(x, w, bias)
    m, k = _rows(x).shape
    n = w.shape[0]
    if w.dtype != x.dtype or not w.is_contiguous() or w.shape[1] != k:
        raise ValueError("linear_dual: weight must be contiguous [N, K] in the activation dtype, K as x")
    m_main = _fused_epilogue_rows(x.dtype, m, n, k, _ld(x))
    if m_main == 0:
        pre = linear(x, w, bias)
        return pre, act_forward(pre, act)
    pre = torch.empty((m, n), dtype=x.dtype, device=x.device)
    y = torch.empty((m, n), dtype=x.dtype, device=x.device)
    with _Timed("linear", flops=2 * m_main * n * k, bytes=(m_main * k + n * k + 2 * m_main * n) * 2, m=m_main, n=n, k=k):
# ... 486 lines not shown
```

anemoi_models_amd/runtime.py:

```python

from __future__ import annotations

import os
from dataclasses import dataclass
from typing import Callable, NamedTuple, Optional, Sequence

import torch
from torch import Tensor

from . import ops

_FORCED_DTYPE = {"fp32": torch.float32, "float32": torch.float32, "bf16": torch.bfloat16,
                 "bfloat16": torch.bfloat16}


def compute_dtype(x: Tensor) -> torch.dtype:
    forced = os.environ.get("ANEMOI_AMD_DTYPE")
    if forced:
        return _FORCED_DTYPE[forced.lower()]
    if torch.is_autocast_enabled():
        dt = torch.get_autocast_dtype("cuda")
        if dt == torch.float16:
            global _FP16_NOTICE
            if not _FP16_NOTICE:
# ... 310 lines not shown
    if edge_index.dim() != 2 or edge_index.shape[0] != 2:
        raise ValueError(f"edge_index must have shape [2, E], got {tuple(edge_index.shape)}")
    e = edge_index.shape[1]
    if e >= 2**31 or n_src >= 2**31 or n_dst >= 2**31:
        raise NotImplementedError("edge / node counts beyond int32 are not supported")
    src, dst = edge_index[0], edge_index[1]
    if e > 0:
        smin, smax = int(src.min()), int(src.max())
        dmin, dmax = int(dst.min()), int(dst.max())
        if smin < 0 or smax >= n_src or dmin < 0 or dmax >= n_dst:
            raise ValueError(
                f"edge_index out of range: src in [{smin}, {smax}] for {n_src} source nodes, "
                f"dst in [{dmin}, {dmax}] for {n_dst} destination nodes"
            )
    perm = torch.argsort(dst, stable=True)
    counts = torch.bincount(dst, minlength=n_dst)
    rowptr = torch.zeros(n_dst + 1, dtype=torch.int64, device=edge_index.device)
    torch.cumsum(counts, 0, out=rowptr[1:])
    return EdgePlan(rowptr.to(torch.int32), src[perm].to(torch.int32).contiguous(), perm.to(torch.int32), n_src,
                    n_dst)


_PLAN_DIR: Optional[str] = None


def set_plan_cache_dir(path: Optional[str]) -> None:
    global _PLAN_DIR
    _PLAN_DIR = path


def plan_cache_dir() -> Optional[str]:
    return _PLAN_DIR or os.environ.get("ANEMOI_AMD_PLAN_CACHE_DIR") or None


def tensor_digest(*items) -> str:
    import hashlib

    h = hashlib.blake2b(digest_size=16)
    for it in items:
        if isinstance(it, Tensor):
            t = it.detach().cpu().contiguous()
            h.update(f"T{t.dtype}{tuple(t.shape)}".encode())
            h.update(t.view(torch.uint8).numpy().tobytes() if t.numel() else b"")
        else:
            h.update(f"V{it!r}".encode())
    return h.hexdigest()


def graph_hash(graph) -> str:
    items = []
    for name, store in sorted(graph.node_items(), key=lambda kv: kv[0]):
        items += ["node", name, store.x]
    edge_types = sorted(graph.edge_types) if hasattr(graph, "edge_types") else []
    for key in edge_types:
        store = graph[key]
        items += ["edge", "/".join(key), store["edge_index"]]
        for k in sorted(k for k in store.keys() if k != "edge_index"):
            v = store[k]
            if isinstance(v, Tensor):
                items += [k, v]
    return tensor_digest(*items)


class PlanCache:

    def __init__(self) -> None:
        self._plans: dict = {}

    @staticmethod
    def _disk_path(edge_index, n_src, n_dst, batch_size, edge_inc, src_map, dst_map) -> Optional[str]:
        root = plan_cache_dir()
        if root is None:
            return None
        key = tensor_digest("edgeplan-v1", edge_index, n_src, n_dst, batch_size, edge_inc if batch_size > 1 else None,
                            src_map, dst_map)
        return os.path.join(root, f"edgeplan-{key}.pt")

    def get(self, edge_index: Tensor, n_src: int, n_dst: int, batch_size: int = 1,
            edge_inc: Optional[Tensor] = None, src_map: Optional[Tensor] = None,
            dst_map: Optional[Tensor] = None) -> EdgePlan:
        key = (edge_index.data_ptr(), edge_index._version, tuple(edge_index.shape), str(edge_index.device), n_src,
               n_dst, batch_size, None if src_map is None else src_map.data_ptr(),
               None if dst_map is None else dst_map.data_ptr())
        plan = self._plans.get(key)
        if plan is None:
            path = self._disk_path(edge_index, n_src, n_dst, batch_size, edge_inc, src_map, dst_map)
            if path is not None and os.path.exists(path):
                plan = load_edge_plan(path, edge_index.device, n_src, n_dst)
            if plan is None:
                ei = edge_index
                if src_map is not None or dst_map is not None:
                    src = ei[0] if src_map is None else src_map[ei[0]]
                    dst = ei[1] if dst_map is None else dst_map[ei[1]]
                    ei = torch.stack([src, dst])
                if batch_size > 1:
                    ei = expand_edges(ei, edge_inc, batch_size)
                plan = build_edge_plan(ei, n_src, n_dst)
                if path is not None:
                    save_edge_plan(plan, path)
            if len(self._plans) > 16:
                self._plans.clear()
            self._plans[key] = plan
        return plan


def save_edge_plan(plan: EdgePlan, path: str) -> None:
    os.makedirs(os.path.dirname(path), exist_ok=True)
    tmp = f"{path}.{os.getpid()}.tmp"
    torch.save({"format": "anemoi_models_amd.EdgePlan/1", "rowptr": plan.rowptr.cpu(), "col": plan.col.cpu(),
                "perm": plan.perm.cpu(), "n_src": plan.n_src, "n_dst": plan.n_dst}, tmp)
    os.replace(tmp, path)


def load_edge_plan(path: str, device, n_src: Optional[int] = None, n_dst: Optional[int] = None) -> Optional[EdgePlan]:
    try:
        d = torch.load(path, map_location="cpu", weights_only=True)
        rowptr, col, perm = d["rowptr"], d["col"], d["perm"]
        n_edges = col.shape[0]
        ok = (d.get("format") == "anemoi_models_amd.EdgePlan/1" and rowptr.dtype == torch.int32
              and col.dtype == torch.int32 and perm.dtype == torch.int32
              and rowptr.dim() == 1 and col.dim() == 1 and rowptr.shape[0] == d["n_dst"] + 1 and col.shape == perm.shape
              and (n_src is None or int(d["n_src"]) == int(n_src)) and (n_dst is None or int(d["n_dst"]) == int(n_dst))
              and int(rowptr[0]) == 0 and int(rowptr[-1]) == n_edges and bool((rowptr[1:] >= rowptr[:-1]).all()))
        if ok and n_edges > 0:
            ok = (int(col.min()) >= 0 and int(col.max()) < int(d["n_src"])
                  and bool((torch.bincount(perm.long().clamp_(0, n_edges - 1), minlength=n_edges) == 1).all())
                  and int(perm.min()) >= 0 and int(perm.max()) < n_edges)
    except Exception:
        return None
    if not ok:
        return None
    return EdgePlan(rowptr.to(device), col.to(device), perm.to(device), int(d["n_src"]), int(d["n_dst"]))


def locality_order(sincos_latlon: Tensor) -> Tensor:
    s_lat, s_lon, c_lat, c_lon = sincos_latlon.detach().double().unbind(dim=1)
    xyz = torch.stack([c_lat * c_lon, c_lat * s_lon, s_lat], dim=1)
    q = ((xyz + 1.0) * 0.5 * 1023.0).round().clamp_(0, 1023).to(torch.int64)
    code = torch.zeros(q.shape[0], dtype=torch.int64, device=q.device)
    for bit in range(10):
        for axis in range(3):
            code |= ((q[:, axis] >> bit) & 1) << (3 * bit + axis)
    return torch.argsort(code, stable=True)


def inverse_permutation(order: Tensor) -> Tensor:
    inv = torch.empty_like(order)
    inv[order] = torch.arange(order.shape[0], device=order.device, dtype=order.dtype)
    return inv


def expand_edges(edge_index: Tensor, edge_inc: Tensor, batch_size: int) -> Tensor:
    return torch.cat([edge_index + i * edge_inc for i in range(batch_size)], dim=1)


class PackedWeights:

    def __init__(self) -> None:
        self._store: dict = {}

    def get(self, key, params: Sequence[Optional[Tensor]], build: Callable[[], Tensor]) -> Tensor:
        ver = tuple((p.data_ptr(), p._version, p.device) for p in params if p is not None)
        hit = self._store.get(key)
        if hit is not None and hit[0] == ver:
            return hit[1]
        with torch.no_grad():
            val = build()
        self._store[key] = (ver, val)
        return val

    def clear(self) -> None:
        self._store.clear()


def edge_attr_csr_cached(cache: PackedWeights, edge_attr: Tensor, trainable: Optional[Tensor], plan, *layout) -> Tensor:
    def build():
        return plan, ops.edge_attr_csr(edge_attr, trainable, plan.perm, *layout)

    return cache.get(("edge_attr_csr", id(plan), layout), [edge_attr, trainable], build)[1]


def pack_weight(weights: Sequence[Tensor], dtype: torch.dtype, k_pad: Optional[int] = None) -> Tensor:
    w = torch.cat([t.detach() for t in weights], dim=0) if len(weights) > 1 else weights[0].detach()
    k = w.shape[1]
    kp = ops.round_up(k, ops.k_multiple(dtype)) if k_pad is None else k_pad
    out = torch.zeros((w.shape[0], kp), dtype=dtype, device=w.device)
    out[:, :k] = w.to(dtype)
    return out


def pack_weight_cols(parts: Sequence[Tensor], dtype: torch.dtype) -> Tensor:
    w = torch.cat([t.detach() for t in parts], dim=1)
    k = w.shape[1]
    kp = ops.round_up(k, ops.k_multiple(dtype))
    out = torch.zeros((w.shape[0], kp), dtype=dtype, device=w.device)
    out[:, :k] = w.to(dtype)
    return out


def ln_fold_enabled(dtype: torch.dtype) -> bool:
    return dtype == torch.bfloat16 and os.environ.get("ANEMOI_AMD_LN_FOLD", "1") != "0"


def fold_layer_norm(w_rows: Tensor, bias: Optional[Tensor], gamma: Tensor, beta: Tensor, dtype: torch.dtype):
    w = w_rows.detach().float()
    g, bt = gamma.detach().float(), beta.detach().float()
    k = w.shape[1]
    kp = ops.round_up(k, ops.k_multiple(dtype))
    wp = torch.zeros((w.shape[0], kp), dtype=dtype, device=w.device)
    wp[:, :k] = (w * g[None, :]).to(dtype)
    colsum = wp.float().sum(dim=1).contiguous()
    b = w @ bt
    if bias is not None:
        b = b + bias.detach().float()
    return wp, b.contiguous(), colsum


def mxfp8_enabled(dtype: torch.dtype) -> bool:
    return dtype == torch.bfloat16 and os.environ.get("ANEMOI_AMD_MXFP8", "0") == "1"


def mx_weight(cache: "PackedWeights", key, params: Sequence[Optional[Tensor]], rows: Callable[[], tuple]):
    def build():
        w, b = rows()
        return ops.mx_quantize(w.detach().float().contiguous()), None if b is None else b.detach().float().contiguous()

    return cache.get(("mxfp8",) + tuple(key), params, build)


def f32_linear_split(dtype: torch.dtype) -> bool:
    mode = os.environ.get("ANEMOI_AMD_F32_LINEAR", "exact")
    if mode not in ("exact", "bf16x3"):
        raise ValueError(f"ANEMOI_AMD_F32_LINEAR={mode!r}: expected 'exact' or 'bf16x3'")
    return mode == "bf16x3" and dtype == torch.float32


def split_route(m: int, n: int, k: int) -> bool:
    return k >= SPLIT_MIN_K


SPLIT_MIN_K = 32


def split_planes(w: Tensor) -> "ops.SplitWeight":
    owner = w._base if w._base is not None else w
    store = owner.__dict__.get("_anemoi_split")
    if store is None:
        store = owner._anemoi_split = {}
    key = (w.storage_offset(), tuple(w.shape), tuple(w.stride()))
    hit = store.get(key)
    if hit is not None and hit[0] == (w.data_ptr(), w._version):
        return hit[1]
    with torch.no_grad():
        planes = ops.split_weight(w)
    store[key] = ((w.data_ptr(), w._version), planes)
# ... 217 lines not shown
```

include/anemoi_amd.h:

```cpp
#ifndef ANEMOI_AMD_H
#define ANEMOI_AMD_H

#include <stdint.h>

#ifdef __cplusplus
extern "C" {
#endif

#define ANEMOI_OK 0
#define ANEMOI_ERR_INVALID 1
#define ANEMOI_ERR_UNSUPPORTED 2
#define ANEMOI_ERR_LAUNCH 3

#define ANEMOI_F32 0
#define ANEMOI_BF16 1
#define ANEMOI_I32 2
#define ANEMOI_U8 3

#define ANEMOI_ACT_NONE 0
#define ANEMOI_ACT_GELU 1
#define ANEMOI_ACT_SILU 2
#define ANEMOI_ACT_RELU 3

typedef void* anemoi_stream_t;
// ... 229 lines not shown
                          int64_t stride_w, void* y, int64_t ldy, int64_t stride_y, int batch, int64_t M, int N, int K,
                          anemoi_stream_t stream);

int64_t anemoi_col_sum_workspace_floats(int64_t rows, int cols);
int anemoi_col_sum(int dtype, const void* x, int64_t ldx, int64_t rows, int cols, float* out, float* workspace,
                   int64_t workspace_floats, anemoi_stream_t stream);

int anemoi_row_dot(int dtype, const void* a, int64_t lda, const void* b, int64_t ldb, const float* shift, float* out,
                   int64_t rows, int cols, anemoi_stream_t stream);

int anemoi_row_scale(int dtype, const void* x, int64_t ldx, const float* s, float alpha, void* out, int64_t ldo,
                     int64_t rows, int cols, anemoi_stream_t stream);

int anemoi_act_forward(int dtype, int act, const void* pre, int64_t ldp, const void* residual, int64_t ldr, void* out,
                       int64_t ldo, int64_t rows, int cols, anemoi_stream_t stream);

int anemoi_act_backward(int dtype, int act, const void* pre, int64_t ldp, const void* dy, int64_t ldd, void* out,
                        int64_t ldo, int64_t rows, int cols, anemoi_stream_t stream);

int anemoi_linear_dual(int dtype, const void* x, int64_t ldx, const void* w, const float* bias, void* pre, int64_t ldp,
                       void* y, int64_t ldy, int64_t M, int N, int K, int act, anemoi_stream_t stream);

int anemoi_linear_actgrad(int dtype, const void* x, int64_t ldx, const void* w, const void* pre, int64_t ldp, void* y,
                          int64_t ldy, int64_t M, int N, int K, int act, anemoi_stream_t stream);

enum {
  ANEMOI_LINEAR_ENTRY_LINEAR = 0,
  ANEMOI_LINEAR_ENTRY_LN = 1,
  ANEMOI_LINEAR_ENTRY_STATS = 2,
  ANEMOI_LINEAR_ENTRY_DUAL = 3,
  ANEMOI_LINEAR_ENTRY_ACTGRAD = 4,
  ANEMOI_LINEAR_ENTRY_BATCHED = 5
};
enum { ANEMOI_LINEAR_KERNEL_NONE = 0, ANEMOI_LINEAR_KERNEL_128 = 1, ANEMOI_LINEAR_KERNEL_PERSISTENT = 2 };
enum {
  ANEMOI_LINEAR_REST_NONE = 0,
  ANEMOI_LINEAR_REST_IN_LAUNCH = 1,
  ANEMOI_LINEAR_REST_SKINNY = 2,
  ANEMOI_LINEAR_REST_128 = 3
};

typedef struct anemoi_linear_args {
  int64_t struct_bytes;
  int32_t entry, dtype, out_dtype, act;
  const void* x;
  const void* w;
  const float* bias;
  const float* colsum;
  const float* stats;
  const void* residual;
  void* y;
  int64_t ldx, ldr, ldy, M;
  int32_t N, K;
  void* workspace;
  int64_t workspace_bytes;
  float* stats_out;
  int64_t stride_x, stride_w, stride_y;
  int32_t batch, reserved;
} anemoi_linear_args;

typedef struct anemoi_linear_route_launch {
  int64_t row0, rows, tiles;
  int32_t mh, blocks, tail_rows;
  int32_t stagger_phases, stagger_unit, reserved;
} anemoi_linear_route_launch;

typedef struct anemoi_linear_route_info {
  int64_t struct_bytes;
  int32_t kernel;
  int32_t n_launches;
  anemoi_linear_route_launch launch[2];
  int64_t main_rows;
  int32_t rest;
  int32_t nt;
  int64_t rest_row0, rest_rows;
  int64_t rs_rows;
  int32_t vec_ok;
  int32_t split;
  int32_t model;
  int32_t reserved;
} anemoi_linear_route_info;

int anemoi_linear_route(const anemoi_linear_args* args, anemoi_linear_route_info* route);

int64_t anemoi_layer_norm_backward_workspace_floats(int64_t rows, int C);
int anemoi_layer_norm_backward(int dtype, const void* x, int64_t ldx, const float* stats, const float* gamma,
                               const void* dy, int64_t ldd, const void* dres, int64_t ldr, void* dx, int64_t ldo,
                               int64_t rows, int C, float* dgamma, float* dbeta, float* workspace,
                               int64_t workspace_floats, anemoi_stream_t stream);

int anemoi_gt_edge_attention_folded_backward_dst(int dtype, const void* q, int64_t ldq, const void* k, const void* v,
                                                 int64_t ldkv, const void* dout, int64_t ldd, const void* u, int64_t ldu,
                                                 const void* dt, int64_t lddt, const float* lse, const float* edge_attr,
                                                 int up, const int32_t* rowptr, const int32_t* col, float* alpha,
                                                 float* w, float* dsum, void* dq, int64_t lddq, void* du, int64_t lddu,
                                                 void* dxr, int64_t lddxr, int64_t n_dst, int C, int H,
                                                 anemoi_stream_t stream);
int anemoi_gt_edge_attention_folded_backward_src(int dtype, const void* q, int64_t ldq, const void* dout, int64_t ldd,
                                                 const float* alpha, const float* w, const float* dsum,
                                                 const int32_t* rowptr_t, const int32_t* eid_t, const int32_t* dst_t,
                                                 void* dk, void* dv, int64_t ldg, int64_t n_src, int C, int H,
                                                 anemoi_stream_t stream);
int anemoi_gt_edge_attr_grad(int dtype, const float* alpha, const float* w, const float* dsum, const void* u, int64_t ldu,
                             const void* dt, int64_t lddt, const int32_t* dst_of_edge, float* dattr, int64_t n_edges,
                             int H, int up, int D, anemoi_stream_t stream);

typedef struct anemoi_gt_block_args {
  int64_t struct_bytes;
  int64_t n_dst;
  int32_t dtype;
  int32_t C, H, up;
  int32_t hidden, act;
  int32_t k_proj, n_in;
  float eps_mlp, eps_out;
  const void* x; int64_t ldx; const float* x_stats;
  const void* w_in; const float* b_in; const float* cs_in;
  void* sq; int64_t ld_sq;
  const void* q; const void* k; const void* v; const void* x_r; const void* u;
  int64_t ldq, ldkv, ldr, ldu;
  const float* edge_attr; const int32_t* rowptr; const int32_t* col;
  void* att; int64_t ld_att;
  const void* w_proj; const float* b_proj; const void* res; int64_t ld_res; void* y; float* y_stats;
  const void* w_fc1; const float* b_fc1; const float* cs_fc1; void* h;
  const void* w_fc2; const float* b_fc2; void* out; float* out_stats;
  void* stats_ws; int64_t stats_ws_bytes;
  const int32_t* run_ptr; const int32_t* run_perm; int64_t n_runs;
  const int32_t* sched; int32_t sched_slots, sched_steps; int64_t n_src;
  const int32_t* run_dst;
  int64_t n_edges;
  const int32_t* tile_hdr; const int32_t* tile_dst; const int32_t* tile_src; const uint8_t* tile_slot; const int32_t* tile_xcd;
  int32_t tile_max_per_xcd, tile_src_cap, tile_edge_cap, tile_pad;
} anemoi_gt_block_args;
int anemoi_gt_block_tail(const anemoi_gt_block_args* args, anemoi_stream_t stream);
int anemoi_gt_processor_block_forward(const anemoi_gt_block_args* args, anemoi_stream_t stream);

typedef struct anemoi_tfm_block_args {
  int64_t struct_bytes;
  int64_t rows;
  int32_t dtype;
  int32_t B, S, C, H;
  int32_t hidden, act;
  int32_t window;
  float eps1, eps2;
  float dropout_p; uint32_t dropout_seed; const void* dropout_seed_dev; int32_t dropout_h0, dropout_h_total;
  const void* x; int64_t ldx;
  const float* ln1_w; const float* ln1_b; const float* ln2_w; const float* ln2_b;
  const void* w_qkv; const float* b_qkv;
  const void* w_proj; const float* b_proj;
  const void* w_fc1; const float* b_fc1;
  const void* w_fc2; const float* b_fc2;
  void* h_ln;
  void* qkv;
  void* att;
  void* y;
  void* h;
  void* mhsa_ws;
  void* out;
} anemoi_tfm_block_args;
int anemoi_transformer_block_forward(const anemoi_tfm_block_args* args, anemoi_stream_t stream);


int anemoi_mx_quantize(int dtype, const void* x, int64_t ldx, const float* gamma, const float* beta, float eps,
                       uint8_t* q, int64_t ldq, uint8_t* s, int64_t lds, int64_t rows, int K, int Kp,
                       anemoi_stream_t stream);

int anemoi_linear_mx(const uint8_t* xq, int64_t ldxq, const uint8_t* xs, int64_t ldxs, const uint8_t* wq,
// ... 128 lines not shown
```

Before: 19.55 million mesh-node updates/s.

## Add thin-GEMM MFMA kernels with fused LN fold, bias, residual and stats

Adds a new HIP kernel family for GEMMs with small fixed N/K shapes (encoder/decoder embeddings and heads). It keeps the weights in registers, streams rows with prefetching, and uses either row-parallel or K-split MFMA layouts. Bias, a LayerNorm fold via row stats and column sums, residual addition and output row-stats are fused into the epilogue. It also adds hoisting and caching helpers. The aim is to cut launch count and memory passes for these thin linears, at the cost of many template instantiations and more routing complexity.

```diff
diff --git a/anemoi_models_amd/_lib.py b/anemoi_models_amd/_lib.py
--- a/anemoi_models_amd/_lib.py
+++ b/anemoi_models_amd/_lib.py
@@ -93,6 +93,23 @@
     for name, value in fields.items():
         setattr(args, name, value)
     return load().anemoi_linear_route(ctypes.byref(args), ctypes.byref(route)), route
+
+
+class LinearThinArgs(ctypes.Structure):
+
+    _fields_ = [
+        ("struct_bytes", c_int64),
+        ("out_dtype", ctypes.c_int32), ("batch", ctypes.c_int32),
+        ("x", c_void_p), ("w", c_void_p), ("bias", c_void_p), ("colsum", c_void_p), ("stats", c_void_p),
+        ("residual", c_void_p), ("y", c_void_p), ("stats_out", c_void_p),
+        ("ldx", c_int64), ("ldr", c_int64), ("ldy", c_int64), ("M", c_int64),
+        ("N", ctypes.c_int32), ("K", ctypes.c_int32),
+        ("stride_x", c_int64), ("stride_w", c_int64), ("stride_y", c_int64), ("stride_r", c_int64),
+        ("eps", c_float), ("reserved", ctypes.c_int32),
+    ]
+
+
+THIN_SHAPES = ((256, 64), (64, 256), (256, 256), (80, 1024), (16, 1024), (16, 256), (256, 128))
 
 
 class GtBlockArgs(ctypes.Structure):
@@ -251,6 +268,7 @@
     "anemoi_linear_dual": (c_int, [c_int, c_void_p, c_int64, c_void_p, c_void_p, c_void_p, c_int64, c_void_p, c_int64,
                                    c_int64, c_int, c_int, c_int, c_void_p]),
     "anemoi_linear_route": (c_int, [ctypes.POINTER(LinearArgs), ctypes.POINTER(LinearRoute)]),
+    "anemoi_linear_thin": (c_int, [ctypes.POINTER(LinearThinArgs), c_void_p]),
     "anemoi_linear_actgrad": (c_int, [c_int, c_void_p, c_int64, c_void_p, c_void_p, c_int64, c_void_p, c_int64, c_int64,
                                       c_int, c_int, c_int, c_void_p]),
     "anemoi_gt_conv": (c_int, [c_int, c_void_p, c_int64, c_void_p, c_void_p, c_int64, c_void_p, c_int64, c_void_p, c_int64,
diff --git a/anemoi_models_amd/csrc/gemm_thin.hip b/anemoi_models_amd/csrc/gemm_thin.hip
--- /dev/null
+++ b/anemoi_models_amd/csrc/gemm_thin.hip
@@ -0,0 +1,444 @@
+
+#include <type_traits>
+
+#include "common.hpp"
+#include "gemm_thin_plan.hpp"
+#include "trail.hpp"
+
+namespace anemoi {
+namespace thin {
+
+typedef __attribute__((ext_vector_type(8))) __bf16 bf16x8_t;
+typedef __attribute__((ext_vector_type(4))) float f32x4_t;
+typedef __attribute__((ext_vector_type(4))) uint32_t u32x4_t;
+
+struct Params {
+  const bf16_t* x;
+  const bf16_t* w;
+  const float* bias;
+  const float* colsum;
+  const float2* stats;
+  const bf16_t* res;
+  void* y;
+  float2* stats_out;
+  int64_t ldx, ldr, ldy, M, row_blocks;
+  int64_t sx, sw, sy, sr;
+  int N;
+  int out_f32, pair;
+  float eps;
+};
+
+template <bool STREAM>
+__device__ __forceinline__ bf16x8_t load_frag(const bf16_t* p) {
+  const u32x4_t* q = reinterpret_cast<const u32x4_t*>(p);
+  if constexpr (STREAM) return __builtin_bit_cast(bf16x8_t, __builtin_nontemporal_load(q));
+  return __builtin_bit_cast(bf16x8_t, *q);
+}
+
+__device__ __forceinline__ int col_of(int j, int q, int pair) {
+  return pair ? (j >> 1) * 32 + q * 8 + (j & 1) * 4 : j * 16 + q * 4;
+}
+
+enum { OUT_BF16 = 0, OUT_F32 = 1, OUT_STATS = 2 };
+
+template <int N>
+__device__ __forceinline__ void fill_table(float (&tab)[2][N], const Params& p, int bias_off) {
+  for (int n = threadIdx.x; n < N; n += 256) {
+    tab[0][n] = p.colsum != nullptr ? p.colsum[n] : 0.f;
+    tab[1][n] = p.bias != nullptr ? p.bias[bias_off + n] : 0.f;
+  }
+  __syncthreads();
+}
+
+__device__ __forceinline__ void finish4(float (&v)[4], bool fold, float2 st, float4 cs, float4 b, bool round) {
+  if (fold) {
+    v[0] = fmaf(v[0], st.x, st.y * cs.x);
+    v[1] = fmaf(v[1], st.x, st.y * cs.y);
+    v[2] = fmaf(v[2], st.x, st.y * cs.z);
+    v[3] = fmaf(v[3], st.x, st.y * cs.w);
+  }
+  v[0] += b.x;
+  v[1] += b.y;
+  v[2] += b.z;
+  v[3] += b.w;
+  if (round) {
+#pragma unroll
+    for (int i = 0; i < 4; ++i) v[i] = bf16_to_f32(f32_to_bf16(v[i]));
+  }
+}
+
+__device__ __forceinline__ void add4(float (&v)[4], uint2 r) {
+  v[0] += __uint_as_float(r.x << 16);
+  v[1] += __uint_as_float(r.x & 0xffff0000u);
+  v[2] += __uint_as_float(r.y << 16);
+  v[3] += __uint_as_float(r.y & 0xffff0000u);
+}
+
+template <int K, int NT, bool NSPLIT, int PF, int OUT, bool RES>
+__global__ __launch_bounds__(256) void thin_rows_kernel(Params p) {
+  constexpr int KF = K / 32, N = NT * 16 * (NSPLIT ? 4 : 1);
+  __shared__ __attribute__((aligned(16))) float tab[2][N];
+  __shared__ float red[2][4][16];
+  const int lane = threadIdx.x & 63, fr = lane & 15, fq = lane >> 4;
+  const int wid = __builtin_amdgcn_readfirstlane((int)(threadIdx.x >> 6));
+  const int64_t h = blockIdx.y;
+  const bf16_t* X = p.x + h * p.sx;
+  const bf16_t* W = p.w + h * p.sw;
+  const int col0 = NSPLIT ? wid * NT * 16 : 0;
+  const int pair = OUT == OUT_BF16 ? p.pair : 0;
+  const bool fold = p.stats != nullptr, round = !p.out_f32;
+  fill_table<N>(tab, p, (int)h * N);
+
+  const int nrb = (int)p.row_blocks;
+  const int first = NSPLIT ? (int)blockIdx.x : (int)blockIdx.x * 4 + wid;
+  const int step = NSPLIT ? (int)gridDim.x : (int)gridDim.x * 4;
+  if (first >= nrb) return;
+
+  bf16x8_t wf[NT][KF];
+#pragma unroll
+  for (int j = 0; j < NT; ++j) {
+    const int n = col0 + col_of(j, fr >> 2, pair) + (fr & 3);
+#pragma unroll
+    for (int ks = 0; ks < KF; ++ks) wf[j][ks] = load_frag<false>(W + (int64_t)n * K + ks * 32 + fq * 8);
+  }
+
+  struct Block {
+    bf16x8_t x[KF];
+    float2 st;
+    uint2 rv[RES ? NT : 1];
+  };
+  Block xb[PF];
+  auto load_block = [&](int rb, Block& dst) {
+    int64_t m = (int64_t)rb * 16 + fr;
+    if (m > p.M - 1) m = p.M - 1;
+    const bf16_t* xr = X + m * p.ldx + fq * 8;
+#pragma unroll
+    for (int ks = 0; ks < KF; ++ks) dst.x[ks] = load_frag<!NSPLIT>(xr + ks * 32);
+    dst.st = *(fold ? p.stats + m : reinterpret_cast<const float2*>(p.w));
+    if constexpr (RES) {
+      const bf16_t* rr = p.res + h * p.sr + m * p.ldr + col0;
+#pragma unroll
+      for (int j = 0; j < NT; ++j) dst.rv[j] = *reinterpret_cast<const uint2*>(rr + col_of(j, fq, pair));
+    }
+  };
+#pragma unroll
+  for (int s = 0; s < PF; ++s) {
+    const int rb = first + s * step;
+    __builtin_amdgcn_sched_barrier(0);
+    load_block(rb < nrb ? rb : first, xb[s]);
+  }
+  __builtin_amdgcn_sched_barrier(0);
+
+  auto process = [&](int rb, Block& xs, auto prefetch) {
+      f32x4_t acc[NT];
+#pragma unroll
+      for (int j = 0; j < NT; ++j) acc[j] = f32x4_t{0.f, 0.f, 0.f, 0.f};
+#pragma unroll
+      for (int ks = 0; ks < KF; ++ks)
+#pragma unroll
+        for (int j = 0; j < NT; ++j) acc[j] = __builtin_amdgcn_mfma_f32_16x16x32_bf16(wf[j][ks], xs.x[ks], acc[j], 0, 0, 0);
+
+      const int64_t m = (int64_t)rb * 16 + fr;
+      const bool valid = m < p.M;
+      const float2 st = xs.st;
+      float v[NT][4];
+#pragma unroll
+      for (int j = 0; j < NT; ++j) {
+        const int n = col0 + col_of(j, fq, pair);
+#pragma unroll
+        for (int i = 0; i < 4; ++i) v[j][i] = acc[j][i];
+        finish4(v[j], fold, st, *reinterpret_cast<const float4*>(&tab[0][n]), *reinterpret_cast<const float4*>(&tab[1][n]), round);
+        if constexpr (RES) add4(v[j], xs.rv[j]);
+      }
+      __builtin_amdgcn_sched_barrier(0);
+      if constexpr (decltype(prefetch)::value) {
+        const int nx = rb + PF * step;
+        load_block(nx < nrb ? nx : rb, xs);
+      }
+      __builtin_amdgcn_sched_barrier(0);
+
+      if constexpr (OUT == OUT_STATS) {
+        float sum = 0.f;
+#pragma unroll
+        for (int j = 0; j < NT; ++j)
+#pragma unroll
+          for (int i = 0; i < 4; ++i) sum += v[j][i];
+        sum += __shfl_xor(sum, 16, 64);
+        sum += __shfl_xor(sum, 32, 64);
+        if constexpr (NSPLIT) {
+          if (fq == 0) red[0][wid][fr] = sum;
+          __syncthreads();
+          sum = ((red[0][0][fr] + red[0][1][fr]) + red[0][2][fr]) + red[0][3][fr];
+        }
+        const float mean = sum / (float)N;
+        float q = 0.f;
+#pragma unroll
+        for (int j = 0; j < NT; ++j)
+#pragma unroll
+          for (int i = 0; i < 4; ++i) {
+            const float d = v[j][i] - mean;
+            q += d * d;
+          }
+        q += __shfl_xor(q, 16, 64);
+        q += __shfl_xor(q, 32, 64);
+        if constexpr (NSPLIT) {
+          if (fq == 0) red[1][wid][fr] = q;
+          __syncthreads();
+          q = ((red[1][0][fr] + red[1][1][fr]) + red[1][2][fr]) + red[1][3][fr];
+        }
+        const float rstd = rsqrtf(q / (float)N + p.eps);
+        if (valid && fq == 0 && (!NSPLIT || wid == 0)) p.stats_out[m] = make_float2(rstd, -mean * rstd);
+      } else {
+        if (valid) {
+          if constexpr (OUT == OUT_F32) {
+            float* yr = static_cast<float*>(p.y) + h * p.sy + m * p.ldy + col0;
+#pragma unroll
+            for (int j = 0; j < NT; ++j) VecIO<float, 4>::store(yr + col_of(j, fq, 0), v[j]);
+          } else {
+            bf16_t* yr = static_cast<bf16_t*>(p.y) + h * p.sy + m * p.ldy + col0;
+            if constexpr (NT % 2 == 0) {
+#pragma unroll
+              for (int j = 0; j < NT; j += 2) {
+                const float o[8] = {v[j][0], v[j][1], v[j][2], v[j][3], v[j + 1][0], v[j + 1][1], v[j + 1][2], v[j + 1][3]};
+                VecIO<bf16_t, 8>::store(yr + col_of(j, fq, 1), o);
+              }
+            } else {
+#pragma unroll
+              for (int j = 0; j < NT; ++j) VecIO<bf16_t, 4>::store(yr + col_of(j, fq, 0), v[j]);
+            }
+          }
+        }
+      }
+  };
+
+  int rb0 = first;
+  for (; rb0 + (PF - 1) * step < nrb; rb0 += PF * step) {
+#pragma unroll
+    for (int s = 0; s < PF; ++s) process(rb0 + s * step, xb[s], std::true_type{});
+  }
+#pragma unroll
+  for (int s = 0; s < PF - 1; ++s)
+    if (rb0 + s * step < nrb) process(rb0 + s * step, xb[s], std::false_type{});
+}
+
+template <int KW, int NT, int PF, int OUT, bool RES>
+__global__ __launch_bounds__(256) void thin_ksplit_kernel(Params p) {
+  constexpr int KF = KW / 32, K = 4 * KW, N = NT * 16, LDP = N + 4, CI = (N + 63) / 64;
+  __shared__ __attribute__((aligned(16))) float part[2][4][16][LDP];
+  __shared__ __attribute__((aligned(16))) float tab[2][N];
+  const int lane = threadIdx.x & 63, fr = lane & 15, fq = lane >> 4;
+  const int wid = __builtin_amdgcn_readfirstlane((int)(threadIdx.x >> 6));
+  const bf16_t* X = p.x + wid * KW;
+  const bf16_t* W = p.w + wid * KW;
+  const bool fold = p.stats != nullptr, round = !p.out_f32;
+  fill_table<N>(tab, p, 0);
+  const int er = threadIdx.x >> 4, ec = (threadIdx.x & 15) * 4;
+
+  bf16x8_t wf[NT][KF];
+#pragma unroll
+  for (int j = 0; j < NT; ++j)
+#pragma unroll
+    for (int ks = 0; ks < KF; ++ks) wf[j][ks] = load_frag<false>(W + (int64_t)(j * 16 + fr) * K + ks * 32 + fq * 8);
+
+  const int nrb = (int)p.row_blocks, first = (int)blockIdx.x, step = (int)gridDim.x;
+  struct Block {
+    bf16x8_t x[KF];
+    float2 st;
+    uint2 rv[RES ? CI : 1];
+  };
+  Block xb[PF];
+  auto load_block = [&](int rb, Block& dst) {
+    int64_t m = (int64_t)rb * 16 + fr;
+    if (m > p.M - 1) m = p.M - 1;
+    const bf16_t* xr = X + m * p.ldx + fq * 8;
+#pragma unroll
+    for (int ks = 0; ks < KF; ++ks) dst.x[ks] = load_frag<true>(xr + ks * 32);
+    int64_t me = (int64_t)rb * 16 + er;
+    if (me > p.M - 1) me = p.M - 1;
+    dst.st = *(fold ? p.stats + me : reinterpret_cast<const float2*>(p.w));
+    if constexpr (RES) {
+#pragma unroll
+      for (int i = 0; i < CI; ++i) dst.rv[i] = *reinterpret_cast<const uint2*>(p.res + me * p.ldr + (ec + i * 64 < N ? ec + i * 64 : 0));
+    }
+  };
+#pragma unroll
+  for (int s = 0; s < PF; ++s) {
+    const int rb = first + s * step;
+    __builtin_amdgcn_sched_barrier(0);
+    load_block(rb < nrb ? rb : first, xb[s]);
+  }
+  __builtin_amdgcn_sched_barrier(0);
+
+  int buf = 0;
+  auto process = [&](int rb, Block& xs, auto prefetch) {
+      f32x4_t acc[NT];
+#pragma unroll
+      for (int j = 0; j < NT; ++j) acc[j] = f32x4_t{0.f, 0.f, 0.f, 0.f};
+#pragma unroll
+      for (int ks = 0; ks < KF; ++ks)
+#pragma unroll
+        for (int j = 0; j < NT; ++j) acc[j] = __builtin_amdgcn_mfma_f32_16x16x32_bf16(wf[j][ks], xs.x[ks], acc[j], 0, 0, 0);
+
+      const int64_t m = (int64_t)rb * 16 + er;
+      const bool valid = m < p.M;
+      const float2 st = xs.st;
+      uint2 rv[RES ? CI : 1];
+      if constexpr (RES) {
+#pragma unroll
+        for (int i = 0; i < CI; ++i) rv[i] = xs.rv[i];
+      }
+      __builtin_amdgcn_sched_barrier(0);
+      if constexpr (decltype(prefetch)::value) {
+        const int nx = rb + PF * step;
+        load_block(nx < nrb ? nx : rb, xs);
+      }
+      __builtin_amdgcn_sched_barrier(0);
+#pragma unroll
+      for (int j = 0; j < NT; ++j)
+        *reinterpret_cast<float4*>(&part[buf][wid][fr][j * 16 + fq * 4]) = make_float4(acc[j][0], acc[j][1], acc[j][2], acc[j][3]);
+      __syncthreads();
+
+      float v[CI][4];
+#pragma unroll
+      for (int i = 0; i < CI; ++i) {
+        const int c = ec + i * 64;
+        if (c < N) {
+          const float4 a0 = *reinterpret_cast<const float4*>(&part[buf][0][er][c]);
+          const float4 a1 = *reinterpret_cast<const float4*>(&part[buf][1][er][c]);
+          const float4 a2 = *reinterpret_cast<const float4*>(&part[buf][2][er][c]);
+          const float4 a3 = *reinterpret_cast<const float4*>(&part[buf][3][er][c]);
+          v[i][0] = ((a0.x + a1.x) + a2.x) + a3.x;
+          v[i][1] = ((a0.y + a1.y) + a2.y) + a3.y;
+          v[i][2] = ((a0.z + a1.z) + a2.z) + a3.z;
+          v[i][3] = ((a0.w + a1.w) + a2.w) + a3.w;
+          finish4(v[i], fold, st, *reinterpret_cast<const float4*>(&tab[0][c]), *reinterpret_cast<const float4*>(&tab[1][c]), round);
+        } else {
+#pragma unroll
+          for (int e = 0; e < 4; ++e) v[i][e] = 0.f;
+        }
+      }
+      buf ^= 1;
+
+      if constexpr (OUT == OUT_STATS) {
+        float sum = 0.f;
+#pragma unroll
+        for (int i = 0; i < CI; ++i)
+          if (ec + i * 64 < N) sum += (v[i][0] + v[i][1]) + (v[i][2] + v[i][3]);
+        const float mean = group_sum<16>(sum) / (float)N;
+        float q = 0.f;
+#pragma unroll
+        for (int i = 0; i < CI; ++i)
+          if (ec + i * 64 < N) {
+#pragma unroll
+            for (int e = 0; e < 4; ++e) {
+              const float d = v[i][e] - mean;
+              q += d * d;
+            }
+          }
+        const float rstd = rsqrtf(group_sum<16>(q) / (float)N + p.eps);
+        if (valid && (threadIdx.x & 15) == 0) p.stats_out[m] = make_float2(rstd, -mean * rstd);
+      } else {
+#pragma unroll
+        for (int i = 0; i < CI; ++i) {
+          const int c = ec + i * 64;
+          if (valid && c < N) {
+            if constexpr (RES) add4(v[i], rv[i]);
+            if constexpr (OUT == OUT_F32)
+              VecIO<float, 4>::store(static_cast<float*>(p.y) + m * p.ldy + c, v[i]);
+            else
+              VecIO<bf16_t, 4>::store(static_cast<bf16_t*>(p.y) + m * p.ldy + c, v[i]);
+          }
+        }
+      }
+  };
+
+  int rb0 = first;
+  for (; rb0 + (PF - 1) * step < nrb; rb0 += PF * step) {
+#pragma unroll
+    for (int s = 0; s < PF; ++s) process(rb0 + s * step, xb[s], std::true_type{});
+  }
+#pragma unroll
+  for (int s = 0; s < PF - 1; ++s)
+    if (rb0 + s * step < nrb) process(rb0 + s * step, xb[s], std::false_type{});
+}
+
+typedef void (*Kernel)(Params);
+#define ANEMOI_THIN_ROWS(K, NT, NS, PF, PFR)                                                                     \
+  {                                                                                                              \
+    thin_rows_kernel<K, NT, NS, PF, OUT_BF16, false>, thin_rows_kernel<K, NT, NS, PF, OUT_F32, false>,           \
+        thin_rows_kernel<K, NT, NS, PF, OUT_STATS, false>, thin_rows_kernel<K, NT, NS, PFR, OUT_BF16, true>,     \
+        thin_rows_kernel<K, NT, NS, PFR, OUT_F32, true>, nullptr                                                 \
+  }
+#define ANEMOI_THIN_KSPLIT(KW, NT, PF)                                                                           \
+  {                                                                                                              \
+    thin_ksplit_kernel<KW, NT, PF, OUT_BF16, false>, thin_ksplit_kernel<KW, NT, PF, OUT_F32, false>,             \
+        thin_ksplit_kernel<KW, NT, PF, OUT_STATS, false>, thin_ksplit_kernel<KW, NT, PF, OUT_BF16, true>,        \
+        thin_ksplit_kernel<KW, NT, PF, OUT_F32, true>, nullptr                                                   \
+  }
+static const Kernel KERNELS[N_SHAPES][6] = {
+    ANEMOI_THIN_ROWS(64, 16, false, 4, 2),
+    ANEMOI_THIN_ROWS(256, 4, false, 4, 4),
+    ANEMOI_THIN_ROWS(256, 4, true, 6, 6),
+    ANEMOI_THIN_KSPLIT(256, 5, 3),
+    ANEMOI_THIN_KSPLIT(256, 1, 3),
+    ANEMOI_THIN_ROWS(256, 1, false, 4, 4),
+    ANEMOI_THIN_ROWS(128, 4, true, 8, 8),
+};
+
+static int device_cus() {
+  static std::atomic<int> cached[256] = {};
+  int dev = 0, cus = 0;
+  if (hipGetDevice(&dev) != hipSuccess) return 0;
+  std::atomic<int>& slot = cached[dev & 255];
+  cus = slot.load(std::memory_order_relaxed);
+  if (cus > 0) return cus;
+  if (hipDeviceGetAttribute(&cus, hipDeviceAttributeMultiprocessorCount, dev) != hipSuccess) return 0;
+  slot.store(cus, std::memory_order_relaxed);
+  return cus;
+}
+
+}
+}
+
+using namespace anemoi;
+
+extern "C" int anemoi_linear_thin(const anemoi_linear_thin_args* args, anemoi_stream_t stream) {
+  thin::Plan pl;
+  int rc = thin::plan(args, thin::device_cus(), pl);
+  if (rc != ANEMOI_OK) return rc;
+  thin::Params p;
+  p.x = static_cast<const bf16_t*>(args->x);
+  p.w = static_cast<const bf16_t*>(args->w);
+  p.bias = args->bias;
+  p.colsum = args->colsum;
+  p.stats = reinterpret_cast<const float2*>(args->stats);
+  p.res = static_cast<const bf16_t*>(args->residual);
+  p.y = args->y;
+  p.stats_out = reinterpret_cast<float2*>(args->stats_out);
+  p.ldx = args->ldx;
+  p.ldr = args->ldr;
+  p.ldy = args->ldy;
+  p.M = args->M;
+  p.row_blocks = pl.row_blocks;
+  const bool batched = args->batch > 1;
+  p.sx = batched ? args->stride_x : 0;
+  p.sw = batched ? args->stride_w : 0;
+  p.sy = batched ? args->stride_y : 0;
+  p.sr = batched ? args->stride_r : 0;
+  p.N = args->N;
+  p.out_f32 = args->out_dtype == ANEMOI_F32;
+  p.pair = pl.pair;
+  p.eps = args->eps;
+  const int out = args->stats_out != nullptr ? thin::OUT_STATS : (p.out_f32 ? thin::OUT_F32 : thin::OUT_BF16);
+  hipLaunchKernelGGL(thin::KERNELS[pl.shape][out + (args->residual != nullptr ? 3 : 0)], dim3(pl.grid_x, pl.grid_y), dim3(256), 0, as_stream(stream), p);
+  rc = check_launch("anemoi_linear_thin");
+  if (args->stats_out != nullptr)
+    return trail::note(rc, "anemoi_linear_thin", "stats", ANEMOI_F32, args->stats_out, 2, args->M, 2, as_stream(stream));
+  if (!batched) return trail::note(rc, "anemoi_linear_thin", "out", args->out_dtype, args->y, args->ldy, args->M, args->N, as_stream(stream));
+  if (trail::armed_state() == nullptr) return rc;
+  const int esz = args->out_dtype == ANEMOI_BF16 ? 2 : 4;
+  for (int b = 0; b < args->batch; ++b)
+    rc = trail::note(rc, "anemoi_linear_thin", "out", args->out_dtype, static_cast<const char*>(args->y) + b * args->stride_y * esz,
+                     args->ldy, args->M, args->N, as_stream(stream));
+  return rc;
+}
diff --git a/anemoi_models_amd/csrc/gemm_thin_plan.hpp b/anemoi_models_amd/csrc/gemm_thin_plan.hpp
--- /dev/null
+++ b/anemoi_models_amd/csrc/gemm_thin_plan.hpp
@@ -0,0 +1,91 @@
+#pragma once
+
+#include "common.hpp"
+
+namespace anemoi {
+namespace thin {
+
+enum Mode { MODE_ROWS = 0, MODE_NSPLIT = 1, MODE_KSPLIT = 2 };
+
+struct Shape {
+  int n, k, mode;
+  int blocks_per_cu;
+};
+
+constexpr Shape SHAPES[] = {
+    {256, 64, MODE_ROWS, 1}, {64, 256, MODE_ROWS, 1}, {256, 256, MODE_NSPLIT, 1}, {80, 1024, MODE_KSPLIT, 1}, {16, 1024, MODE_KSPLIT, 1},
+    {16, 256, MODE_ROWS, 1},  {256, 128, MODE_NSPLIT, 1},
+};
+constexpr int N_SHAPES = (int)(sizeof(SHAPES) / sizeof(SHAPES[0]));
+
+struct Plan {
+  int shape;
+  int pair;
+  int64_t row_blocks;
+  unsigned grid_x, grid_y;
+};
+
+inline bool mult(int64_t v, int64_t m) { return v % m == 0; }
+
+inline int plan(const anemoi_linear_thin_args* a, int cus, Plan& p) {
+  ANEMOI_REQUIRE(a != nullptr, ANEMOI_ERR_INVALID, "anemoi_linear_thin: null argument block");
+  ANEMOI_REQUIRE(a->struct_bytes == (int64_t)sizeof(anemoi_linear_thin_args), ANEMOI_ERR_INVALID,
+                 "anemoi_linear_thin: argument block out of sync with the library (%lld bytes, expected %lld)",
+                 (long long)a->struct_bytes, (long long)sizeof(anemoi_linear_thin_args));
+  ANEMOI_REQUIRE(a->out_dtype == ANEMOI_BF16 || a->out_dtype == ANEMOI_F32, ANEMOI_ERR_INVALID,
+                 "anemoi_linear_thin: out_dtype %d", a->out_dtype);
+  ANEMOI_REQUIRE(a->M >= 0 && a->N > 0 && a->K > 0 && a->batch >= 0, ANEMOI_ERR_INVALID,
+                 "anemoi_linear_thin: M=%lld N=%d K=%d batch=%d", (long long)a->M, a->N, a->K, a->batch);
+  const int batch = a->batch > 1 ? a->batch : 1;
+  const bool stats_only = a->stats_out != nullptr;
+  const bool fold = a->colsum != nullptr || a->stats != nullptr;
+  int shape = -1;
+  for (int i = 0; i < N_SHAPES; ++i)
+    if (SHAPES[i].n == a->N && SHAPES[i].k == a->K) shape = i;
+  ANEMOI_REQUIRE(shape >= 0, ANEMOI_ERR_UNSUPPORTED, "anemoi_linear_thin: no register-resident kernel for N=%d K=%d", a->N, a->K);
+  ANEMOI_REQUIRE(a->M > 0, ANEMOI_ERR_UNSUPPORTED, "anemoi_linear_thin: M = 0");
+  ANEMOI_REQUIRE(a->M <= ((int64_t)1 << 34), ANEMOI_ERR_UNSUPPORTED, "anemoi_linear_thin: M=%lld (more than 2^30 row blocks)", (long long)a->M);
+  ANEMOI_REQUIRE(batch == 1 || (SHAPES[shape].mode != MODE_KSPLIT && !fold && !stats_only), ANEMOI_ERR_UNSUPPORTED,
+                 "anemoi_linear_thin: batch=%d with a K-split shape, a LayerNorm fold or statistics", batch);
+  ANEMOI_REQUIRE(batch <= 65535, ANEMOI_ERR_UNSUPPORTED, "anemoi_linear_thin: batch=%d", batch);
+  ANEMOI_REQUIRE(!(stats_only && a->residual != nullptr), ANEMOI_ERR_UNSUPPORTED,
+                 "anemoi_linear_thin: statistics only with a residual");
+  ANEMOI_REQUIRE((a->colsum != nullptr) == (a->stats != nullptr), ANEMOI_ERR_INVALID,
+                 "anemoi_linear_thin: the LayerNorm fold needs both colsum and stats");
+  ANEMOI_REQUIRE(a->x != nullptr && a->w != nullptr && (stats_only || a->y != nullptr), ANEMOI_ERR_INVALID,
+                 "anemoi_linear_thin: null pointer");
+  const int64_t width_x = (int64_t)a->K, width_y = (int64_t)a->N;
+  ANEMOI_REQUIRE(a->ldx >= width_x && (stats_only || a->ldy >= width_y) && (a->residual == nullptr || a->ldr >= width_y),
+                 ANEMOI_ERR_INVALID, "anemoi_linear_thin: leading dimension below the row width");
+  if (batch > 1) {
+    ANEMOI_REQUIRE(a->stride_x >= 0 && a->stride_w >= 0 && a->stride_y >= 0 && a->stride_r >= 0, ANEMOI_ERR_INVALID,
+                   "anemoi_linear_thin: negative problem stride");
+    ANEMOI_REQUIRE(mult(a->stride_x, 8) && mult(a->stride_w, 8), ANEMOI_ERR_INVALID,
+                   "anemoi_linear_thin: stride_x / stride_w must be multiples of 8 elements");
+  }
+  const int out_mult = a->out_dtype == ANEMOI_BF16 ? 8 : 4;
+  ANEMOI_REQUIRE(aligned16(a->x) && aligned16(a->w) && mult(a->ldx, 8), ANEMOI_ERR_INVALID,
+                 "anemoi_linear_thin: x / w must be 16-byte aligned, ldx a multiple of 8");
+  ANEMOI_REQUIRE(stats_only || (aligned16(a->y) && mult(a->ldy, out_mult) && (batch == 1 || mult(a->stride_y, out_mult))),
+                 ANEMOI_ERR_INVALID, "anemoi_linear_thin: y must be 16-byte aligned, ldy / stride_y multiples of %d", out_mult);
+  ANEMOI_REQUIRE(a->residual == nullptr || (aligned16(a->residual) && mult(a->ldr, 8) && (batch == 1 || mult(a->stride_r, 8))),
+                 ANEMOI_ERR_INVALID, "anemoi_linear_thin: residual must be 16-byte aligned, ldr / stride_r multiples of 8");
+  ANEMOI_REQUIRE(aligned16(a->bias) && aligned16(a->colsum) && ((uintptr_t)a->stats & 7) == 0 && ((uintptr_t)a->stats_out & 7) == 0,
+                 ANEMOI_ERR_INVALID, "anemoi_linear_thin: bias / colsum must be 16-byte aligned, stats 8-byte aligned");
+  ANEMOI_REQUIRE(cus > 0, ANEMOI_ERR_INVALID, "anemoi_linear_thin: %d compute units", cus);
+
+  const Shape& s = SHAPES[shape];
+  p.shape = shape;
+  const int tiles_per_wave = s.n / 16 / (s.mode == MODE_NSPLIT ? 4 : 1);
+  p.pair = (s.mode != MODE_KSPLIT && tiles_per_wave % 2 == 0 && a->out_dtype == ANEMOI_BF16 && !stats_only) ? 1 : 0;
+  p.row_blocks = (a->M + 15) / 16;
+  const int64_t items = s.mode == MODE_ROWS ? (p.row_blocks + 3) / 4 : p.row_blocks;
+  int64_t per_problem = ((int64_t)cus * s.blocks_per_cu + batch - 1) / batch;
+  if (per_problem < 1) per_problem = 1;
+  p.grid_x = (unsigned)(items < per_problem ? items : per_problem);
+  p.grid_y = (unsigned)batch;
+  return ANEMOI_OK;
+}
+
+}
+}
diff --git a/anemoi_models_amd/layers/block.py b/anemoi_models_amd/layers/block.py
--- a/anemoi_models_amd/layers/block.py
+++ b/anemoi_models_amd/layers/block.py
@@ -69,7 +69,9 @@
         t = self._packed.get((self._tag, "embstats", self.dtype, kp, self.one_col), [self.emb.weight, self.emb.bias],
                              lambda: runtime.embedding_stats_operator(self.emb.weight, self.emb.bias, kp, self.one_col,
                                                                       self.dtype))
-        return ops.row_stats(runtime.linear(self.x_aug, t, None, stats_eps=eps), eps)
+        thin = ops.thin_enabled() and os.environ.get("ANEMOI_AMD_THIN_STATS", "0") == "1"
+        st = ops.linear_thin(self.x_aug, t, stats_eps=eps) if thin else None
+        return st if st is not None else ops.row_stats(runtime.linear(self.x_aug, t, None, stats_eps=eps), eps)
 
 
 class BaseBlock(nn.Module, ABC):
@@ -641,11 +643,24 @@
         up = self.fold_width(dtype)
         sq_layers = [self.lin_self, self.lin_query]
         wp, bp = self._folded_out(dtype, up)
-        sq = self._ln_linear(self._ln_begin(self.layer_norm2, x_dst), "squ",
-                             lambda: self._folded_in("squ", sq_layers, dtype, up),
-                             lambda: self._folded_rows(sq_layers, up), self._fold_params(sq_layers))
         per_head = w_qt.dim() == 3
-        qt = ops.linear_heads(sq[:, c:2 * c], w_qt) if per_head else runtime.linear(sq[:, c:2 * c], w_qt)
+
+        def dst_side():
+            sq = self._ln_linear(self._ln_begin(self.layer_norm2, x_dst), "squ",
+                                 lambda: self._folded_in("squ", sq_layers, dtype, up),
+                                 lambda: self._folded_rows(sq_layers, up), self._fold_params(sq_layers))
+            return sq, (ops.linear_heads(sq[:, c:2 * c], w_qt) if per_head else runtime.linear(sq[:, c:2 * c], w_qt))
+
+        sources = runtime.static_sources(x_dst) if runtime.enc_hoist_enabled() else None
+        if sources is not None:
+            ln1, ln2, emb = self.layer_norm1, self.layer_norm2, x_src.emb
+            sources = (sources + [h_dst, ln2.weight, ln2.bias] + self._fold_params(sq_layers)
+                       + [self.lin_key.weight, self.lin_key.bias, self.lin_value.weight, self.lin_value.bias, ln1.weight,
+                          ln1.bias, emb.weight, emb.bias])
+            sq, qt = runtime.hoisted(self._packed, ("squ|qt", dtype, tuple(h_dst.shape), up, x_src.x_aug.shape[1], x_src.one_col),
+                                     sources, dst_side)
+        else:
+            sq, qt = dst_side()
         att = torch.empty((sq.shape[0], wp.shape[1]), dtype=dtype, device=sq.device)
         if wp.shape[1] > c + h * up:
             att[:, c + h * up:].zero_()
@@ -653,8 +668,7 @@
                                       plan.col, h, self.out_channels_conv, up, sum_col, att[:, c:c + h * up])
         del qt
         if per_head:
-            ops.linear_heads(g, w_g, out=att[:, :c])
-            ops.add(att[:, :c], sq[:, :c], out=att[:, :c])
+            ops.linear_heads(g, w_g, out=att[:, :c], residual=sq[:, :c])
         else:
             runtime.linear(g, w_g, residual=sq[:, :c], out=att[:, :c])
         del g
diff --git a/anemoi_models_amd/layers/mapper.py b/anemoi_models_amd/layers/mapper.py
--- a/anemoi_models_amd/layers/mapper.py
+++ b/anemoi_models_amd/layers/mapper.py
@@ -137,11 +137,16 @@
         self._packed = runtime.PackedWeights()
         self._plans = runtime.PlanCache()
 
-    def _embed(self, x_src: Tensor, x_dst: Tensor, one_cols=(None, None)):
+    def _embed(self, x_src: Tensor, x_dst: Tensor, one_cols=(None, None), dst_static: bool = False):
         return x_src, x_dst
 
     def _embedded(self, tag: str, lin: nn.Linear, x: Tensor, eps: Optional[float], one_col: Optional[int],
-                  materialise: bool):
+                  materialise: bool, static: bool = False):
+        sources = runtime.static_sources(x) if static else None
+        if sources is not None:
+            sources = sources + [x, lin.weight, lin.bias]
+            return runtime.hoisted(self._packed, (tag, x.dtype, tuple(x.shape), one_col, eps, materialise), sources,
+                                   lambda: runtime.mark_static(self._embedded(tag, lin, x, eps, one_col, materialise), sources))
         k_in = lin.in_features
         if eps is None or not runtime.embed_fold_enabled(x.dtype) or 2 * (k_in + 1) > lin.out_features:
             return linear_native(self._packed, tag, lin, x, stats_eps=eps)
@@ -176,8 +181,8 @@
         plan = self._plans.get(self.edge_index_base, n_src, n_dst, batch_size, self.edge_inc, src_map, dst_map)
         ea = runtime.edge_attr_csr_cached(self._packed, self.edge_attr, self.trainable.trainable, plan,
                                           *self.proc.edge_layout(x_dst.dtype))
-        h_src, h_dst = self._embed(x_src, x_dst, one_cols)
         num_chunks = self.proc.num_chunks if self.training else inference_num_chunks()
+        h_src, h_dst = self._embed(x_src, x_dst, one_cols, dst_static=num_chunks <= 1 and runtime.enc_hoist_enabled())
         _, h_dst = self.proc.native(h_src, h_dst, ea, plan, num_chunks, out_stats_eps=self._extract_ln_eps(h_dst.dtype))
         return self._extract(h_dst, out_dtype)
 
@@ -244,11 +249,12 @@
                          src_grid_size=src_grid_size, dst_grid_size=dst_grid_size)
         self.emb_nodes_src = nn.Linear(self.in_channels_src, self.hidden_dim)
 
-    def _embed(self, x_src: Tensor, x_dst: Tensor, one_cols=(None, None)):
+    def _embed(self, x_src: Tensor, x_dst: Tensor, one_cols=(None, None), dst_static: bool = False):
         eps1, eps2 = self._block_ln_eps(x_src.dtype)
         return (self._embedded("emb_nodes_src", self.emb_nodes_src, x_src, eps1, one_cols[0],
                                materialise=self.proc.update_src_nodes),
-                self._embedded("emb_nodes_dst", self.emb_nodes_dst, x_dst, eps2, one_cols[1], materialise=True))
+                self._embedded("emb_nodes_dst", self.emb_nodes_dst, x_dst, eps2, one_cols[1], materialise=True,
+                               static=dst_static))
 
     def forward(self, x, batch_size: int, shard_shapes, model_comm_group=None):
         x_dst = self._run(x, batch_size, shard_shapes, model_comm_group)
@@ -281,7 +287,7 @@
         return (x_src, self._apply_module(self.emb_nodes_dst, x_dst), change_channels_in_shape(shapes_src, self.hidden_dim),
                 change_channels_in_shape(shapes_dst, self.hidden_dim))
 
-    def _embed(self, x_src: Tensor, x_dst: Tensor, one_cols=(None, None)):
+    def _embed(self, x_src: Tensor, x_dst: Tensor, one_cols=(None, None), dst_static: bool = False):
         return x_src, self._embedded("emb_nodes_dst", self.emb_nodes_dst, x_dst, self._block_ln_eps(x_dst.dtype)[1],
                                      one_cols[1], materialise=True)
 
@@ -291,7 +297,9 @@
             wf, bf, cs = self._packed.get(("extract", "lnfold", x_dst.dtype), [lin.weight, lin.bias, ln.weight, ln.bias],
                                           lambda: runtime.fold_layer_norm(lin.weight.detach().float(), lin.bias,
                                                                           ln.weight, ln.bias, x_dst.dtype))
-            return runtime.linear(x_dst, wf, bf, out_dtype=out_dtype, ln=(ops.row_stats(x_dst, ln.eps), cs))
+            fold = (ops.row_stats(x_dst, ln.eps), cs)
+            y = ops.linear_thin(x_dst, wf, bf, out_dtype=out_dtype, ln=fold) if ops.thin_enabled() else None
+            return y if y is not None else runtime.linear(x_dst, wf, bf, out_dtype=out_dtype, ln=fold)
         h = ops.layer_norm(x_dst, runtime.f32c(ln.weight), runtime.f32c(ln.bias), ln.eps)
         return linear_native(self._packed, "extract", lin, h, out_dtype=out_dtype)
 
diff --git a/anemoi_models_amd/models/encoder_processor_decoder.py b/anemoi_models_amd/models/encoder_processor_decoder.py
--- a/anemoi_models_amd/models/encoder_processor_decoder.py
+++ b/anemoi_models_amd/models/encoder_processor_decoder.py
@@ -84,6 +84,7 @@
             ]
         )
         self._idx_cache: dict = {}
+        self._hoisted = runtime.PackedWeights()
         self._set_truncation(truncation_data)
 
     def _set_truncation(self, truncation_data) -> None:
@@ -271,13 +272,22 @@
         order, inv = self._mesh_order(x.device)
         tr_hidden = na.trainable_tensors[hidden].trainable
         w_hidden = na.attr_ndims[hidden]
-        x_hidden = ops.assemble_nodes(None, na.latlons(hidden)[order],
+        one_data, one_hidden = (width, w_hidden) if fold else (None, None)
+
+        def hidden_rows():
+            return ops.assemble_nodes(None, na.latlons(hidden)[order],
                                       self._with_ones(None if tr_hidden is None else tr_hidden[order], order.numel(), fold),
                                       batch_size, dtype, ld_out=self._feature_ld(w_hidden + int(fold), dtype, fold))
-        one_data, one_hidden = (width, w_hidden) if fold else (None, None)
-
-        enc = self.encoder.native(x_data, x_hidden, batch_size, dst_map=inv,
-                                  **self._one_cols(self.encoder, one_data, one_hidden))
+
+        enc_kw = self._one_cols(self.encoder, one_data, one_hidden)
+        if runtime.enc_hoist_enabled() and enc_kw:
+            sources = [tr_hidden, na.latlons(hidden), order]
+            x_hidden = runtime.hoisted(self._hoisted, ("x_hidden", dtype, batch_size, str(x.device), fold), sources,
+                                       lambda: runtime.mark_static(hidden_rows(), sources))
+        else:
+            x_hidden = hidden_rows()
+
+        enc = self.encoder.native(x_data, x_hidden, batch_size, dst_map=inv, **enc_kw)
         x_data_latent, x_latent = (x_data, enc) if not isinstance(enc, tuple) else enc
         cond = self._processor_condition(batch_size, x_latent)
         x_proc = (self.processor.native(x_latent, batch_size, node_map=inv) if cond is None
diff --git a/anemoi_models_amd/ops.py b/anemoi_models_amd/ops.py
--- a/anemoi_models_amd/ops.py
+++ b/anemoi_models_amd/ops.py
@@ -1,6 +1,8 @@
 
 from __future__ import annotations
 
+import ctypes
+import os
 from typing import NamedTuple
 from typing import Optional
 
@@ -15,10 +17,11 @@
 
 
 class _Timed:
-    __slots__ = ("name", "work", "start")
+    __slots__ = ("name", "work", "start", "launched")
 
     def __init__(self, name: str, **work) -> None:
         self.name, self.work, self.start = name, work, None
+        self.launched = True
 
     def __enter__(self):
         if PROFILE is not None:
@@ -27,7 +30,7 @@
         return self
 
     def __exit__(self, *exc):
-        if self.start is not None:
+        if self.start is not None and self.launched:
             end = torch.cuda.Event(enable_timing=True)
             end.record(torch.cuda.current_stream())
             PROFILE.append((self.name, self.start, end, self.work))
@@ -458,8 +461,12 @@
     return out
 
 
-def linear_heads(x: Tensor, w: Tensor, out: Optional[Tensor] = None) -> Tensor:
-    _dev(x, w, out)
+def linear_heads(x: Tensor, w: Tensor, out: Optional[Tensor] = None, residual: Optional[Tensor] = None) -> Tensor:
+    _dev(x, w, out, residual)
+    if thin_enabled() and w.dim() == 3:
+        y = linear_thin(x, w, out=out, residual=residual)
+        if y is not None:
+            return y
     _rows(x)
     if w.dim() != 3 or w.dtype != x.dtype or not w.is_contiguous():
         raise ValueError("linear_heads: weight must be contiguous [H, N, K] in the activation dtype")
@@ -479,7 +486,79 @@
         st = _lib.load().anemoi_linear_batched(code, code, x.data_ptr(), _ld(x), k, w.data_ptr(), n * k, out.data_ptr(),
                                                _ld(out), n, h, m, n, k, _stream())
     _lib.check(st, "anemoi_linear_batched")
-    return out
+    if residual is not None:
+        add(out[:, :h * n], residual[:, :h * n], out=out[:, :h * n])
+    return out
+
+
+def thin_enabled() -> bool:
+    return os.environ.get("ANEMOI_AMD_THIN", "1") != "0"
+
+
+def linear_thin(x: Tensor, w: Tensor, bias: Optional[Tensor] = None, *, residual: Optional[Tensor] = None,
+                out: Optional[Tensor] = None, out_dtype: Optional[torch.dtype] = None, ln=None,
+                stats_eps: Optional[float] = None) -> Optional[Tensor]:
+    if not x.is_cuda:
+        return None
+    _dev(x, w, bias, residual, out)
+    _rows(x)
+    if x.dtype != torch.bfloat16 or w.dtype != torch.bfloat16 or not w.is_contiguous() or w.dim() not in (2, 3):
+        return None
+    h = w.shape[0] if w.dim() == 3 else 1
+    n, k = w.shape[-2], w.shape[-1]
+    m = x.shape[0]
+    if (n, k) not in _lib.THIN_SHAPES or m == 0 or x.shape[1] < h * k:
+        return None
+    odt = out.dtype if out is not None else (out_dtype or x.dtype)
+    if odt not in _DT:
+        return None
+    mult = 8 if odt == torch.bfloat16 else 4
+    for t, md in ((x, 8), (w, 8), (out, mult), (residual, 8)):
+        if t is not None and (t.data_ptr() % 16 != 0 or (t.dim() == 2 and _ld(_rows(t)) % md != 0)):
+            return None
+    for t in (bias,) + (tuple(ln) if ln is not None else ()):
+        if t is not None and t.data_ptr() % 16 != 0:
+            return None
+    a = _lib.LinearThinArgs()
+    a.struct_bytes = ctypes.sizeof(_lib.LinearThinArgs)
+    a.out_dtype, a.batch = _DT[odt], h
+    a.x, a.w, a.bias = x.data_ptr(), w.data_ptr(), _ptr(bias)
+    a.ldx, a.M, a.N, a.K = _ld(x), m, n, k
+    a.stride_x, a.stride_w, a.stride_y, a.stride_r = k, n * k, n, n
+    if bias is not None and (bias.dtype != torch.float32 or not bias.is_contiguous() or bias.numel() < h * n):
+        raise ValueError("linear_thin: bias must be a contiguous f32 vector with one entry per output column")
+    if ln is not None:
+        stats, colsum = ln
+        _dev(stats, colsum)
+        if stats.shape != (m, 2) or stats.dtype != torch.float32 or not stats.is_contiguous():
+            raise ValueError("linear_thin: ln stats must be the contiguous [M, 2] f32 result of row_stats(x)")
+        if colsum.numel() < n or colsum.dtype != torch.float32 or not colsum.is_contiguous():
+            raise ValueError("linear_thin: ln colsum must be a contiguous f32 vector with one entry per output column")
+        a.stats, a.colsum = stats.data_ptr(), colsum.data_ptr()
+    if residual is not None:
+        if residual.dtype != torch.bfloat16 or _rows(residual).shape[0] != m or residual.shape[1] < h * n:
+            raise ValueError("linear_thin: the residual must be bf16 [M, >= H*N]")
+        a.residual, a.ldr = residual.data_ptr(), _ld(residual)
+    result = None
+    if stats_eps is not None:
+        result = torch.empty((m, 2), dtype=torch.float32, device=x.device)
+        a.stats_out, a.eps = result.data_ptr(), stats_eps
+        moved = (m * h * k + h * n * k) * 2 + m * 8
+    else:
+        if out is None:
+            out = torch.empty((m, h * n), dtype=odt, device=x.device)
+        if _rows(out).shape[0] != m or out.shape[1] < h * n:
+            raise ValueError("linear_thin: out must be [M, >= H*N]")
+        result = out
+        a.y, a.ldy = out.data_ptr(), _ld(out)
+        moved = (m * h * k + h * n * k) * 2 + m * h * n * (out.element_size() + (0 if residual is None else 2))
+    with _Timed("linear", flops=2 * m * h * n * k, bytes=moved, m=m, n=h * n, k=k, thin=True) as timed:
+        st = _lib.load().anemoi_linear_thin(ctypes.byref(a), _stream())
+        timed.launched = st == _lib.ANEMOI_OK
+    if st == _lib.ANEMOI_ERR_UNSUPPORTED:
+        return None
+    _lib.check(st, "anemoi_linear_thin")
+    return result
 
 
 def gt_edge_attention_raw(qt: Tensor, x_raw: Tensor, src_stats: Tensor, u: Tensor, edge_attr: Tensor, rowptr: Tensor,
@@ -1132,8 +1211,9 @@
         raise ValueError("add: shape / dtype mismatch")
     if out is None:
         out = torch.empty(a.shape, dtype=a.dtype, device=a.device)
-    st = _lib.load().anemoi_add(dtype_code(a.dtype), a.data_ptr(), _ld(_rows(a)), b.data_ptr(), _ld(_rows(b)),
-                                out.data_ptr(), _ld(_rows(out)), a.shape[0], a.shape[1], _stream())
+    with _Timed("add", bytes=3 * a.shape[0] * a.shape[1] * a.element_size(), m=a.shape[0], n=a.shape[1]):
+        st = _lib.load().anemoi_add(dtype_code(a.dtype), a.data_ptr(), _ld(_rows(a)), b.data_ptr(), _ld(_rows(b)),
+                                    out.data_ptr(), _ld(_rows(out)), a.shape[0], a.shape[1], _stream())
     _lib.check(st, "anemoi_add")
     return out
 
diff --git a/anemoi_models_amd/runtime.py b/anemoi_models_amd/runtime.py
--- a/anemoi_models_amd/runtime.py
+++ b/anemoi_models_amd/runtime.py
@@ -416,7 +416,7 @@
         key = (edge_index.data_ptr(), edge_index._version, tuple(edge_index.shape), str(edge_index.device), n_src,
                n_dst, batch_size, None if src_map is None else src_map.data_ptr(),
                None if dst_map is None else dst_map.data_ptr())
-        plan = self._plans.get(key)
+        plan = self._plans.get(key, (None,))[0]
         if plan is None:
             path = self._disk_path(edge_index, n_src, n_dst, batch_size, edge_inc, src_map, dst_map)
             if path is not None and os.path.exists(path):
@@ -434,7 +434,7 @@
                     save_edge_plan(plan, path)
             if len(self._plans) > 16:
                 self._plans.clear()
-            self._plans[key] = plan
+            self._plans[key] = (plan, src_map, dst_map)
         return plan
 
 
@@ -505,6 +505,28 @@
 
     def clear(self) -> None:
         self._store.clear()
+
+
+ROUTE_SWITCHES = ("ANEMOI_AMD_THIN", "ANEMOI_AMD_THIN_STATS", "ANEMOI_AMD_LN_FOLD", "ANEMOI_AMD_EMBED_FOLD", "ANEMOI_AMD_EDGE_RAW", "ANEMOI_AMD_EDGE_FOLD",
+                  "ANEMOI_AMD_F32_LINEAR", "ANEMOI_AMD_MXFP8")
+
+
+def enc_hoist_enabled() -> bool:
+    return os.environ.get("ANEMOI_AMD_ENC_HOIST", "1") != "0" and not torch.is_grad_enabled()
+
+
+def hoisted(cache: PackedWeights, key, sources: Sequence[Optional[Tensor]], build: Callable[[], object]):
+    switches = tuple(os.environ.get(name) for name in ROUTE_SWITCHES)
+    return cache.get(("hoist", key, switches), sources, lambda: ([s for s in sources if s is not None], build()))[1]
+
+
+def static_sources(t) -> Optional[list]:
+    return getattr(t, "_anemoi_static", None)
+
+
+def mark_static(t, sources: Sequence[Optional[Tensor]]):
+    t._anemoi_static = [s for s in sources if s is not None]
+    return t
 
 
 def edge_attr_csr_cached(cache: PackedWeights, edge_attr: Tensor, trainable: Optional[Tensor], plan, *layout) -> Tensor:
diff --git a/include/anemoi_amd.h b/include/anemoi_amd.h
--- a/include/anemoi_amd.h
+++ b/include/anemoi_amd.h
@@ -335,6 +335,27 @@
 } anemoi_linear_route_info;
 
 int anemoi_linear_route(const anemoi_linear_args* args, anemoi_linear_route_info* route);
+
+typedef struct anemoi_linear_thin_args {
+  int64_t struct_bytes;
+  int32_t out_dtype;
+  int32_t batch;
+  const void* x;
+  const void* w;
+  const float* bias;
+  const float* colsum;
+  const float* stats;
+  const void* residual;
+  void* y;
+  float* stats_out;
+  int64_t ldx, ldr, ldy, M;
+  int32_t N, K;
+  int64_t stride_x, stride_w, stride_y, stride_r;
+  float eps;
+  int32_t reserved;
+} anemoi_linear_thin_args;
+
+int anemoi_linear_thin(const anemoi_linear_thin_args* args, anemoi_stream_t stream);
 
 int64_t anemoi_layer_norm_backward_workspace_floats(int64_t rows, int C);
 int anemoi_layer_norm_backward(int dtype, const void* x, int64_t ldx, const float* stats, const float* gamma,
```

New measurement: 20.00 million mesh-node updates/s (median of 6 runs). 2.3% higher.
